# nloyfer/wgbs_tools

Measured on AMD Instinct MI355X. Metric: CpG-sites/sec segmented, higher is better.
Workload: dtype u8 counts -> u32 prefix sums -> f32/f64 log-likelihood (bit-exact with the reference)

## Files before the change

### include/wgbsseg.h

```cpp
#ifndef WGBSSEG_H
#define WGBSSEG_H

#include <stddef.h>
#include <stdint.h>

#ifdef __cplusplus
extern "C" {
#endif

#define WGBSSEG_VERSION 290
#define WGBSSEG_MAX_CPG 65535

#define WGBSSEG_OK              0
#define WGBSSEG_E_ARG          -1
#define WGBSSEG_E_METH_GT_COV  -2
#define WGBSSEG_E_NOMEM        -3
#define WGBSSEG_E_HIP          -4
#define WGBSSEG_E_LOCI_ORDER   -5
#define WGBSSEG_E_CAPACITY     -6
#define WGBSSEG_E_STATE        -7
#define WGBSSEG_E_IO           -8

typedef struct wgbsseg_ctx wgbsseg_ctx;

typedef struct wgbsseg_params {
    float    pseudo_count;
    uint32_t max_cpg;
    uint32_t max_bp;
} wgbsseg_params;

typedef struct wgbsseg_timings {
    double scan_ms;
    double window_ms;
    double cost_ms;
    double dp_ms;
    double trace_ms;
    double total_ms;
    int64_t sites;
    int64_t pairs;
    int64_t evals;
    int64_t scan_bytes;
    int32_t max_window;
    int32_t n_stages;
    int32_t scan_launches;
    int32_t div_short;
    double  scan_main_ms;
    int64_t scan_main_bytes;
} wgbsseg_timings;

int wgbsseg_version(void);

int wgbsseg_device_count(void);

int wgbsseg_create(int device, wgbsseg_ctx** out, char* err, size_t errlen);
void wgbsseg_destroy(wgbsseg_ctx* ctx);

int wgbsseg_set_betas_host(wgbsseg_ctx* ctx, const uint8_t* const* samples, int64_t n_samples, int64_t n_sites,
                           char* err, size_t errlen);
int wgbsseg_set_lbetas_host(wgbsseg_ctx* ctx, const uint16_t* const* samples, int64_t n_samples, int64_t n_sites,
                            char* err, size_t errlen);
int wgbsseg_set_betas_device(wgbsseg_ctx* ctx, const void* base, int64_t n_samples, int64_t pitch_bytes,
                             int64_t n_sites, char* err, size_t errlen);

int wgbsseg_set_loci_host(wgbsseg_ctx* ctx, const uint32_t* loci, int64_t n_sites, char* err, size_t errlen);
int wgbsseg_set_loci_device(wgbsseg_ctx* ctx, const void* loci, int64_t n_sites, char* err, size_t errlen);

int wgbsseg_segment_chunks(wgbsseg_ctx* ctx, const int64_t* chunk_start0, const int32_t* chunk_len,
                           int64_t n_chunks, const wgbsseg_params* params,
                           int32_t* borders_out, int64_t borders_cap, int64_t* borders_off,
                           char* err, size_t errlen);

int wgbsseg_segment_regions(wgbsseg_ctx* ctx, const int64_t* region_start, const int64_t* region_end, int64_t n_regions,
                            int64_t chunk_size, const wgbsseg_params* params,
                            int32_t* borders_out, int64_t borders_cap, int64_t* borders_off, int64_t* stats,
                            char* err, size_t errlen);

typedef int (*wgbsseg_batch_fn)(void* user, const int64_t* starts, const int64_t* ends, int64_t n,
                                const int32_t** out_ptr, int64_t* out_cnt);
int wgbsseg_stitch_regions(const int64_t* region_start, const int64_t* region_end, int64_t n_regions, int64_t chunk_size,
                           wgbsseg_batch_fn fn, void* user, int32_t speculate, int32_t* borders_out, int64_t borders_cap,
                           int64_t* borders_off, int64_t* stats, char* err, size_t errlen);

int wgbsseg_first_batch_items(const int64_t* region_start, const int64_t* region_end, int64_t n_regions, int64_t chunk_size,
                              int32_t speculate, int64_t* starts, int64_t* ends, int64_t cap, int64_t* n_items, int64_t* n_chunks,
                              char* err, size_t errlen);

int wgbsseg_set_site_base(wgbsseg_ctx* ctx, int64_t site_base);

typedef struct wgbsseg_group wgbsseg_group;
int wgbsseg_plan_shares(const uint32_t* loci, int64_t n_sites, const int64_t* region_start, const int64_t* region_end,
                        int64_t n_regions, int64_t chunk_size, const wgbsseg_params* params, int32_t n_shares, int64_t halo,
                        int64_t* own_lo, int64_t* own_hi, int64_t* win_lo, int64_t* win_hi, int64_t* share_chunks,
                        int64_t* share_work, char* err, size_t errlen);
// ... 68 lines not shown
                     const wgbsseg_bed_opts* opts, int fd, int64_t* lines_written, int64_t* bytes_written,
                     char* err, size_t errlen);
void wgbsseg_beta2bed_pass_ms(const wgbsseg_ctx* ctx, double* length_ms, double* emit_ms);
void wgbsseg_beta2bed_limits(int64_t* default_slab, int64_t* max_slab, int32_t* max_stage_bytes, int32_t* max_name);

int wgbsseg_site_counts(wgbsseg_ctx* ctx, const int64_t* site0, int64_t n_rows, const int32_t* samples, int32_t n_cols,
                        uint16_t* out, char* err, size_t errlen);
typedef struct {
    int32_t min_cov;
    int32_t reserved;
    int64_t slab_rows;
} wgbsseg_site_table_opts;
int wgbsseg_site_table(wgbsseg_ctx* ctx, const int64_t* site0, int64_t n_rows, const int32_t* samples, int32_t n_cols,
                       const char* labels, const int64_t* label_off, const wgbsseg_site_table_opts* opts, int fd,
                       int64_t* lines_written, int64_t* bytes_written, char* err, size_t errlen);
void wgbsseg_site_table_pass_ms(const wgbsseg_ctx* ctx, double* gather_ms, double* length_ms, double* emit_ms);
void wgbsseg_site_table_limits(int64_t* default_slab_rows, int64_t* max_slab_rows, int32_t* max_label, int32_t* max_cols);

int wgbsseg_convert_regions(wgbsseg_ctx* ctx, const int64_t* chrom_lo, const int64_t* chrom_hi, const int64_t* chrom_bp,
                            const int64_t* start, const int64_t* end, const uint8_t* slow, int64_t n,
                            int64_t* start_cpg, int64_t* end_cpg, char* err, size_t errlen);

int wgbsseg_add_loci(const uint32_t* loci, int64_t n_sites, const int64_t* chrom_cum, const char* const* chrom_names,
                     int32_t n_chroms, const int64_t* start_cpg, const int64_t* end_cpg, int64_t n_blocks,
                     const char* path, int32_t append, int32_t threads, char* err, size_t errlen);

int wgbsseg_add_loci_borders(const uint32_t* loci, int64_t n_sites, const int64_t* chrom_cum, const char* const* chrom_names,
                             int32_t n_chroms, const int32_t* borders, const int64_t* borders_off, int64_t n_regions,
                             int64_t min_cpg, const char* path, int32_t append, int32_t threads,
                             int64_t* n_written, int64_t* n_dropped, char* err, size_t errlen);

int wgbsseg_blocks_parse(const char* text, int64_t len, int64_t max_rows, int64_t cap, int64_t* line_off, int32_t* len3,
                         int64_t* start_cpg, int64_t* end_cpg, uint8_t* na, int64_t* n_rows,
                         int64_t* bp_start, int64_t* bp_end, int32_t* bp_ok, int32_t* first_fields);
int wgbsseg_blocks_write_table(const char* path, int32_t append, const char* text, const int64_t* line_off, const int32_t* len3,
                               const int64_t* start_cpg, const int64_t* end_cpg, const uint8_t* na, int64_t n_rows,
                               const double* values, int64_t n_cols, int64_t stride, int32_t digits, int32_t threads, char* err, size_t errlen);
int wgbsseg_blocks_write_bedgraph(const char* path, const char* text, const int64_t* line_off, const int32_t* len3, int64_t n_rows,
                                  const void* rows, int32_t wide, int32_t threads, char* err, size_t errlen);
int64_t wgbsseg_format_fixed(const double* v, int64_t n, int32_t digits, char* out, int64_t out_cap);

int wgbsseg_bed_parse(const char* text, int64_t len, int64_t cap, const char* const* chrom_names, int32_t n_chroms, int64_t* line_off,
                      int32_t* len3, int32_t* row_len, int32_t* chrom, int64_t* start, int64_t* end, int64_t* n_rows, int32_t* width, int32_t* header);
int64_t wgbsseg_debug_canonical_float(const char* tokens, int64_t len, uint8_t* out, int64_t out_cap);
int wgbsseg_bed_write_annotated(const char* path, const char* text, const int64_t* line_off, const int32_t* len3, const int32_t* row_len,
                                const int64_t* start_cpg, const int64_t* end_cpg, int64_t n_rows, int32_t threads, char* err, size_t errlen);

typedef struct wgbsseg_patbeta wgbsseg_patbeta;
int wgbsseg_patbeta_create(int device, int64_t start_cpg, int64_t end_cpg, wgbsseg_patbeta** out, char* err, size_t errlen);
int wgbsseg_patbeta_feed(wgbsseg_patbeta* pb, const char* text, int64_t n_bytes, char* err, size_t errlen);
int wgbsseg_patbeta_finish(wgbsseg_patbeta* pb, int32_t lbeta, void* out, char* err, size_t errlen);
void wgbsseg_patbeta_destroy(wgbsseg_patbeta* pb);
double wgbsseg_patbeta_kernel_ms(wgbsseg_patbeta* pb);

typedef struct wgbsseg_homog wgbsseg_homog;
int wgbsseg_homog_create(int device, const int64_t* start_cpg, const int64_t* end_cpg, int64_t n_blocks, const float* range, int32_t n_bins,
                         int32_t min_cpgs, int32_t inclusive, wgbsseg_homog** out, char* err, size_t errlen);
int wgbsseg_homog_feed(wgbsseg_homog* h, const char* text, int64_t n_bytes, char* err, size_t errlen);
int wgbsseg_homog_finish(wgbsseg_homog* h, int32_t* counts, char* err, size_t errlen);
void wgbsseg_homog_destroy(wgbsseg_homog* h);
double wgbsseg_homog_kernel_ms(wgbsseg_homog* h);
int wgbsseg_debug_homog_bins(const float* range, int32_t n_bins, int32_t max_total, int8_t* out);

typedef struct wgbsseg_bimodal wgbsseg_bimodal;
int wgbsseg_bimodal_create(int device, const int64_t* start_cpg, const int64_t* end_cpg, int64_t n_blocks, int32_t strict, int32_t min_len,
                           int32_t max_lds_cols, wgbsseg_bimodal** out, char* err, size_t errlen);
int wgbsseg_bimodal_feed(wgbsseg_bimodal* b, const char* text, int64_t n_bytes, char* err, size_t errlen);
int wgbsseg_bimodal_finish(wgbsseg_bimodal* b, double* ll, int64_t* counts, char* err, size_t errlen);
void wgbsseg_bimodal_destroy(wgbsseg_bimodal* b);
double wgbsseg_bimodal_kernel_ms(wgbsseg_bimodal* b);
int wgbsseg_debug_bimodal_terms(const uint32_t* a, const uint32_t* b, int64_t count, uint64_t* out);

int wgbsseg_patbeta_feed_bgzf(wgbsseg_patbeta* pb, const void* bytes, int64_t n_bytes, int64_t* consumed, char* err, size_t errlen);
int wgbsseg_homog_feed_bgzf(wgbsseg_homog* h, const void* bytes, int64_t n_bytes, int64_t* consumed, char* err, size_t errlen);
int wgbsseg_bimodal_feed_bgzf(wgbsseg_bimodal* b, const void* bytes, int64_t n_bytes, int64_t* consumed, char* err, size_t errlen);
double wgbsseg_patbeta_inflate_ms(wgbsseg_patbeta* pb);
double wgbsseg_homog_inflate_ms(wgbsseg_homog* h);
double wgbsseg_bimodal_inflate_ms(wgbsseg_bimodal* b);
int wgbsseg_bgzf_inflate(int device, const void* bytes, int64_t n_bytes, void* out, int64_t out_cap, int64_t* out_len, int64_t* consumed,
                         char* err, size_t errlen);

int wgbsseg_get_timings(const wgbsseg_ctx* ctx, wgbsseg_timings* out);

int64_t wgbsseg_debug_fetch(wgbsseg_ctx* ctx, const char* what, void* out, int64_t cap_bytes);
int wgbsseg_debug_sample_terms(wgbsseg_ctx* ctx, const float* nmeth, const float* ntotal, int64_t count,
                               float pseudo_count, float* out);
int wgbsseg_debug_log2(wgbsseg_ctx* ctx, uint32_t first_bits, int64_t count, uint32_t* out_f, uint64_t* out_d,
                       uint64_t* out_fast);
int wgbsseg_debug_div(wgbsseg_ctx* ctx, const float* a, const float* b, int64_t count, uint32_t* out_fast, uint32_t* out_ieee);
int wgbsseg_debug_check_div(wgbsseg_ctx* ctx, float pseudo_count, int32_t max_total, int64_t* mismatches);
int wgbsseg_debug_div_short(wgbsseg_ctx* ctx, const float* a, const float* b, int64_t count, uint32_t* out);

#ifdef __cplusplus
}
#endif
#endif
```

### wgbs_tools_amd/_lib.py

```python
import ctypes as C
import os
import os.path as op

import numpy as np

HERE = op.dirname(op.abspath(__file__))
LIB_PATH = op.join(HERE, 'csrc', 'libwgbsseg.so')
if os.environ.get('WGBSSEG_LIB') and os.environ.get('WGBSSEG_ALLOW_LIB_OVERRIDE') == '1':
    LIB_PATH = os.environ['WGBSSEG_LIB']
    import sys as _sys
    print('[wgbsseg] WGBSSEG_LIB: loading %s instead of the in-tree library' % LIB_PATH, file=_sys.stderr)
SYNTH_LIB_PATH = op.join(HERE, 'csrc', 'libwgbssynth.so')

OK, E_ARG, E_METH_GT_COV, E_NOMEM, E_HIP, E_LOCI_ORDER, E_CAPACITY, E_STATE, E_IO = 0, -1, -2, -3, -4, -5, -6, -7, -8

ABI_VERSION = 290
EXPORTS = ['wgbsseg_version', 'wgbsseg_device_count', 'wgbsseg_create', 'wgbsseg_destroy',
           'wgbsseg_set_betas_host', 'wgbsseg_set_betas_device', 'wgbsseg_set_loci_host', 'wgbsseg_set_loci_device',
           'wgbsseg_segment_chunks', 'wgbsseg_segment_regions', 'wgbsseg_segment_chunks_host', 'wgbsseg_prefix_sums', 'wgbsseg_scan_only',
           'wgbsseg_get_timings', 'wgbsseg_debug_fetch', 'wgbsseg_debug_sample_terms', 'wgbsseg_debug_log2',
           'wgbsseg_debug_div', 'wgbsseg_debug_check_div', 'wgbsseg_debug_div_short', 'wgbsseg_add_loci', 'wgbsseg_add_loci_borders', 'wgbsseg_block_sums', 'wgbsseg_last_block_sums_ms',
           'wgbsseg_set_site_base', 'wgbsseg_stitch_regions', 'wgbsseg_group_create', 'wgbsseg_group_destroy', 'wgbsseg_group_size',
           'wgbsseg_group_plan', 'wgbsseg_group_load_host', 'wgbsseg_group_share_set_device', 'wgbsseg_group_segment_regions', 'wgbsseg_group_segment_region_range',
           'wgbsseg_group_get_timings', 'wgbsseg_plan_shares', 'wgbsseg_set_lbetas_host',
           'wgbsseg_convert_regions', 'wgbsseg_patbeta_create', 'wgbsseg_patbeta_feed', 'wgbsseg_patbeta_finish',
           'wgbsseg_patbeta_destroy', 'wgbsseg_patbeta_kernel_ms', 'wgbsseg_group_load_host_async', 'wgbsseg_group_load_wait',
           'wgbsseg_marker_stats', 'wgbsseg_blocks_parse', 'wgbsseg_blocks_write_table', 'wgbsseg_blocks_write_bedgraph',
           'wgbsseg_format_fixed', 'wgbsseg_bed_parse', 'wgbsseg_bed_write_annotated', 'wgbsseg_debug_canonical_float',
           'wgbsseg_first_batch_items', 'wgbsseg_plan_shares_weighted',
           'wgbsseg_homog_create', 'wgbsseg_homog_feed', 'wgbsseg_homog_finish', 'wgbsseg_homog_destroy', 'wgbsseg_homog_kernel_ms',
           'wgbsseg_debug_homog_bins',
           'wgbsseg_bimodal_create', 'wgbsseg_bimodal_feed', 'wgbsseg_bimodal_finish', 'wgbsseg_bimodal_destroy', 'wgbsseg_bimodal_kernel_ms',
           'wgbsseg_debug_bimodal_terms', 'wgbsseg_sample_stats',
           'wgbsseg_pair_ranges', 'wgbsseg_pair_hist', 'wgbsseg_pair_hist_limits',
           'wgbsseg_beta2bed', 'wgbsseg_beta2bed_pass_ms', 'wgbsseg_beta2bed_limits',
           'wgbsseg_site_counts', 'wgbsseg_site_table', 'wgbsseg_site_table_pass_ms', 'wgbsseg_site_table_limits',
           'wgbsseg_patbeta_feed_bgzf', 'wgbsseg_homog_feed_bgzf', 'wgbsseg_bimodal_feed_bgzf',
           'wgbsseg_patbeta_inflate_ms', 'wgbsseg_homog_inflate_ms', 'wgbsseg_bimodal_inflate_ms', 'wgbsseg_bgzf_inflate']


class NativeLibraryError(RuntimeError):
    pass


class SegmentorError(RuntimeError):

    def __init__(self, code, msg):
        super().__init__('[wgbsseg %d] %s' % (code, msg))
        self.code = code
        self.msg = msg


class Params(C.Structure):
    _fields_ = [('pseudo_count', C.c_float), ('max_cpg', C.c_uint32), ('max_bp', C.c_uint32)]


SAMPLE_STAT_DTYPE = np.dtype([('n_sites', np.uint64), ('meth_sum', np.uint64), ('cov_sum', np.uint64), ('covered', np.uint64),
                              ('covered_at', np.uint64), ('orphans', np.uint64), ('ratio_lo', np.uint64), ('ratio_hi', np.uint64),
                              ('max_cov', np.uint32), ('reserved', np.uint32)])

PAIR_RANGE_DTYPE = np.dtype([('n', np.uint64), ('a_min', np.float64), ('a_max', np.float64), ('b_min', np.float64), ('b_max', np.float64)])


class BedOpts(C.Structure):
    _fields_ = [('min_cov', C.c_int32), ('mean', C.c_int32), ('keep_na', C.c_int32), ('stage_bytes', C.c_int32), ('slab_sites', C.c_int64)]


class SiteTableOpts(C.Structure):
    _fields_ = [('min_cov', C.c_int32), ('reserved', C.c_int32), ('slab_rows', C.c_int64)]


class Timings(C.Structure):
    _fields_ = [('scan_ms', C.c_double), ('window_ms', C.c_double), ('cost_ms', C.c_double), ('dp_ms', C.c_double),
                ('trace_ms', C.c_double), ('total_ms', C.c_double), ('sites', C.c_int64), ('pairs', C.c_int64),
                ('evals', C.c_int64), ('scan_bytes', C.c_int64), ('max_window', C.c_int32), ('n_stages', C.c_int32),
                ('scan_launches', C.c_int32), ('div_short', C.c_int32), ('scan_main_ms', C.c_double),
                ('scan_main_bytes', C.c_int64)]

    def as_dict(self):
        return {k: getattr(self, k) for k, _ in self._fields_}


BATCH_FN = C.CFUNCTYPE(C.c_int, C.c_void_p, C.POINTER(C.c_int64), C.POINTER(C.c_int64), C.c_int64, C.POINTER(C.c_void_p),
                       C.POINTER(C.c_int64))

_lib = None
_synth = None
ERRLEN = 512
_hip_preloaded = False


def _share_hip_runtime_with_torch():
    global _hip_preloaded
    if _hip_preloaded:
        return
    _hip_preloaded = True
    import importlib.util
    import sys
    if 'torch' in sys.modules:
        return
    try:
        spec = importlib.util.find_spec('torch')
    except (ImportError, ValueError):
        spec = None
    if spec is None or not spec.origin:
        return
    cand = op.join(op.dirname(spec.origin), 'lib', 'libamdhip64.so')
    if op.isfile(cand):
        try:
            C.CDLL(cand, mode=C.RTLD_GLOBAL)
        except OSError:
            pass


def load():
    global _lib
    if _lib is not None:
        return _lib
    if not op.isfile(LIB_PATH):
        raise NativeLibraryError('%s is missing: build it with `python -m wgbs_tools_amd.build` (needs hipcc). '
                                 'There is no CPU fallback.' % LIB_PATH)
    _share_hip_runtime_with_torch()
    L = C.CDLL(LIB_PATH)
    vp, i64, i32 = C.c_void_p, C.c_int64, C.c_int
    L.wgbsseg_version.restype = i32
    got = L.wgbsseg_version()
    if got != ABI_VERSION:
        raise NativeLibraryError('%s reports ABI version %d, this binding was written against %d (include/wgbsseg.h WGBSSEG_VERSION): '
                                 'rebuild it with `python -m wgbs_tools_amd.build -f`' % (LIB_PATH, got, ABI_VERSION))
    L.wgbsseg_device_count.restype = i32
    L.wgbsseg_create.restype = i32
    L.wgbsseg_create.argtypes = [i32, C.POINTER(vp), C.c_char_p, C.c_size_t]
    L.wgbsseg_destroy.restype = None
    L.wgbsseg_destroy.argtypes = [vp]
    L.wgbsseg_set_betas_host.restype = i32
    L.wgbsseg_set_betas_host.argtypes = [vp, C.POINTER(vp), i64, i64, C.c_char_p, C.c_size_t]
    L.wgbsseg_set_lbetas_host.restype = i32
    L.wgbsseg_set_lbetas_host.argtypes = [vp, C.POINTER(vp), i64, i64, C.c_char_p, C.c_size_t]
    L.wgbsseg_set_betas_device.restype = i32
    L.wgbsseg_set_betas_device.argtypes = [vp, vp, i64, i64, i64, C.c_char_p, C.c_size_t]
    L.wgbsseg_set_loci_host.restype = i32
    L.wgbsseg_set_loci_host.argtypes = [vp, vp, i64, C.c_char_p, C.c_size_t]
    L.wgbsseg_set_loci_device.restype = i32
    L.wgbsseg_set_loci_device.argtypes = [vp, vp, i64, C.c_char_p, C.c_size_t]
    L.wgbsseg_segment_chunks.restype = i32
    L.wgbsseg_segment_chunks.argtypes = [vp, vp, vp, i64, C.POINTER(Params), vp, i64, vp, C.c_char_p, C.c_size_t]
    L.wgbsseg_segment_regions.restype = i32
    L.wgbsseg_segment_regions.argtypes = [vp, vp, vp, i64, i64, C.POINTER(Params), vp, i64, vp, vp, C.c_char_p, C.c_size_t]
    L.wgbsseg_segment_chunks_host.restype = i32
    L.wgbsseg_segment_chunks_host.argtypes = [vp, i64, i64, i64, vp, vp, vp, i64, C.POINTER(Params), i32, vp, i64, vp,
                                              C.c_char_p, C.c_size_t]
    L.wgbsseg_prefix_sums.restype = i32
    L.wgbsseg_prefix_sums.argtypes = [vp, i64, i64, vp, C.c_char_p, C.c_size_t]
    L.wgbsseg_scan_only.restype = i32
    L.wgbsseg_scan_only.argtypes = [vp, vp, vp, i64, i32, i32, C.POINTER(C.c_double), C.POINTER(i64), C.POINTER(i64), C.c_char_p, C.c_size_t]
    L.wgbsseg_get_timings.restype = i32
    L.wgbsseg_get_timings.argtypes = [vp, C.POINTER(Timings)]
    L.wgbsseg_debug_fetch.restype = i64
    L.wgbsseg_debug_fetch.argtypes = [vp, C.c_char_p, vp, i64]
    L.wgbsseg_debug_sample_terms.restype = i32
    L.wgbsseg_debug_sample_terms.argtypes = [vp, vp, vp, i64, C.c_float, vp]
    L.wgbsseg_debug_log2.restype = i32
    L.wgbsseg_debug_log2.argtypes = [vp, C.c_uint32, i64, vp, vp, vp]
    L.wgbsseg_debug_div_short.restype = i32
    L.wgbsseg_debug_div_short.argtypes = [vp, vp, vp, i64, vp]
    L.wgbsseg_debug_check_div.restype = i32
    L.wgbsseg_debug_check_div.argtypes = [vp, C.c_float, i32, vp]
    L.wgbsseg_debug_div.restype = i32
    L.wgbsseg_debug_div.argtypes = [vp, vp, vp, i64, vp, vp]
    L.wgbsseg_block_sums.restype = i32
    L.wgbsseg_block_sums.argtypes = [vp, vp, vp, i64, i32, C.c_uint32, vp, C.c_char_p, C.c_size_t]
    L.wgbsseg_last_block_sums_ms.restype = C.c_double
    L.wgbsseg_last_block_sums_ms.argtypes = [vp]
    L.wgbsseg_sample_stats.restype = i32
    L.wgbsseg_sample_stats.argtypes = [vp, vp, vp, i64, i32, vp, C.c_char_p, C.c_size_t]
    L.wgbsseg_pair_ranges.restype = i32
    L.wgbsseg_pair_ranges.argtypes = [vp, vp, vp, i64, i32, vp, C.c_char_p, C.c_size_t]
    L.wgbsseg_pair_hist.restype = i32
    L.wgbsseg_pair_hist.argtypes = [vp, vp, vp, i64, i32, i32, vp, vp, C.c_char_p, C.c_size_t]
    L.wgbsseg_pair_hist_limits.restype = None
    L.wgbsseg_pair_hist_limits.argtypes = [vp, vp]
    L.wgbsseg_beta2bed.restype = i32
    L.wgbsseg_beta2bed.argtypes = [vp, i32, i64, i64, vp, vp, C.POINTER(C.c_char_p), i32, C.POINTER(BedOpts), C.c_int, vp, vp, C.c_char_p, C.c_size_t]
    L.wgbsseg_beta2bed_pass_ms.restype = None
    L.wgbsseg_beta2bed_pass_ms.argtypes = [vp, vp, vp]
    L.wgbsseg_beta2bed_limits.restype = None
    L.wgbsseg_beta2bed_limits.argtypes = [vp, vp, vp, vp]
    L.wgbsseg_site_counts.restype = i32
    L.wgbsseg_site_counts.argtypes = [vp, vp, i64, vp, i32, vp, C.c_char_p, C.c_size_t]
    L.wgbsseg_site_table.restype = i32
    L.wgbsseg_site_table.argtypes = [vp, vp, i64, vp, i32, vp, vp, C.POINTER(SiteTableOpts), C.c_int, vp, vp, C.c_char_p, C.c_size_t]
    L.wgbsseg_site_table_pass_ms.restype = None
    L.wgbsseg_site_table_pass_ms.argtypes = [vp, vp, vp, vp]
    L.wgbsseg_site_table_limits.restype = None
    L.wgbsseg_site_table_limits.argtypes = [vp, vp, vp, vp]
    L.wgbsseg_set_site_base.restype = i32
    L.wgbsseg_set_site_base.argtypes = [vp, i64]
    L.wgbsseg_stitch_regions.restype = i32
    L.wgbsseg_stitch_regions.argtypes = [vp, vp, i64, i64, BATCH_FN, vp, i32, vp, i64, vp, vp, C.c_char_p, C.c_size_t]
    L.wgbsseg_first_batch_items.restype = i32
    L.wgbsseg_first_batch_items.argtypes = [vp, vp, i64, i64, i32, vp, vp, i64, C.POINTER(i64), C.POINTER(i64), C.c_char_p, C.c_size_t]
    L.wgbsseg_plan_shares.restype = i32
    L.wgbsseg_plan_shares.argtypes = [vp, i64, vp, vp, i64, i64, C.POINTER(Params), i32, i64, vp, vp, vp, vp, vp, vp, C.c_char_p, C.c_size_t]
    L.wgbsseg_plan_shares_weighted.restype = i32
    L.wgbsseg_plan_shares_weighted.argtypes = [vp, i64, vp, vp, i64, i64, C.POINTER(Params), i32, vp, i64, vp, vp, vp, vp, vp, vp, C.c_char_p, C.c_size_t]
    L.wgbsseg_group_create.restype = i32
    L.wgbsseg_group_create.argtypes = [vp, i32, C.POINTER(vp), C.c_char_p, C.c_size_t]
    L.wgbsseg_group_destroy.restype = None
    L.wgbsseg_group_destroy.argtypes = [vp]
    L.wgbsseg_group_size.restype = i32
    L.wgbsseg_group_size.argtypes = [vp]
    L.wgbsseg_group_plan.restype = i32
    L.wgbsseg_group_plan.argtypes = [vp, vp, i64, vp, vp, i64, i64, C.POINTER(Params), i64, vp, vp, vp, vp, C.c_char_p, C.c_size_t]
    L.wgbsseg_group_load_host.restype = i32
    L.wgbsseg_group_load_host.argtypes = [vp, C.POINTER(vp), i64, i64, C.c_char_p, C.c_size_t]
    L.wgbsseg_group_load_host_async.restype = i32
    L.wgbsseg_group_load_host_async.argtypes = [vp, C.POINTER(vp), i64, i64, C.c_char_p, C.c_size_t]
    L.wgbsseg_group_load_wait.restype = i32
    L.wgbsseg_group_load_wait.argtypes = [vp, C.c_char_p, C.c_size_t]
    L.wgbsseg_group_share_set_device.restype = i32
    L.wgbsseg_group_share_set_device.argtypes = [vp, i32, vp, i64, i64, C.c_char_p, C.c_size_t]
    L.wgbsseg_group_segment_regions.restype = i32
    L.wgbsseg_group_segment_regions.argtypes = [vp, vp, i64, vp, vp, C.c_char_p, C.c_size_t]
    L.wgbsseg_group_segment_region_range.restype = i32
    L.wgbsseg_group_segment_region_range.argtypes = [vp, i64, i64, vp, i64, vp, vp, C.c_char_p, C.c_size_t]
    L.wgbsseg_group_get_timings.restype = i32
    L.wgbsseg_group_get_timings.argtypes = [vp, i32, C.POINTER(Timings)]
    L.wgbsseg_convert_regions.restype = i32
    L.wgbsseg_convert_regions.argtypes = [vp, vp, vp, vp, vp, vp, vp, i64, vp, vp, C.c_char_p, C.c_size_t]
    L.wgbsseg_patbeta_create.restype = i32
    L.wgbsseg_patbeta_create.argtypes = [i32, i64, i64, C.POINTER(vp), C.c_char_p, C.c_size_t]
    L.wgbsseg_patbeta_feed.restype = i32
    L.wgbsseg_patbeta_feed.argtypes = [vp, C.c_char_p, i64, C.c_char_p, C.c_size_t]
    L.wgbsseg_patbeta_finish.restype = i32
    L.wgbsseg_patbeta_finish.argtypes = [vp, i32, vp, C.c_char_p, C.c_size_t]
    L.wgbsseg_patbeta_destroy.restype = None
    L.wgbsseg_patbeta_destroy.argtypes = [vp]
    L.wgbsseg_patbeta_kernel_ms.restype = C.c_double
    L.wgbsseg_patbeta_kernel_ms.argtypes = [vp]
    L.wgbsseg_homog_create.restype = i32
# ... 240 lines not shown
        _check(self._L.wgbsseg_pair_ranges(self._h, a.ctypes.data, b.ctypes.data, a.size, int(min_cov), out.ctypes.data, self._err, ERRLEN), self._err)
        return out

    def pair_hist(self, pairs, min_cov, bins, edges):
        a, b = self._pair_columns(pairs)
        bins = int(bins)
        e = np.ascontiguousarray(edges, dtype=np.float64)
        if a.size and bins >= 1 and e.size != a.size * 2 * (bins + 1):
            raise ValueError('pair_hist: edges must hold [n_pairs = %d][2][bins + 1 = %d] doubles, got %d' % (a.size, bins + 1, e.size))
        counts = np.zeros((a.size, max(bins, 0), max(bins, 0)), dtype=np.uint64)
        _check(self._L.wgbsseg_pair_hist(self._h, a.ctypes.data, b.ctypes.data, a.size, int(min_cov), bins, e.ctypes.data, counts.ctypes.data,
                                         self._err, ERRLEN), self._err)
        return counts

    def beta2bed(self, fd, sample, chrom_names, chrom_cum, start0=0, end0=None, mult=None, min_cov=1, mean=False, keep_na=False,
                 slab_sites=0, stage_bytes=0):
        end0 = self.n_sites if end0 is None else int(end0)
        cum = np.ascontiguousarray(chrom_cum, dtype=np.int64)
        names = (C.c_char_p * len(chrom_names))(*[str(n).encode() for n in chrom_names])
        m = None
        if mult is not None:
            m = np.ascontiguousarray(mult, dtype=np.uint16)
            if m.size != max(end0 - int(start0), 0):
                raise ValueError('beta2bed: mult must hold one count per site of [start0, end0): %d for %d sites' % (m.size, end0 - int(start0)))
        opts = BedOpts(int(min_cov), int(bool(mean)), int(bool(keep_na)), int(stage_bytes), int(slab_sites))
        lines, nbytes = C.c_int64(0), C.c_int64(0)
        rc = self._L.wgbsseg_beta2bed(self._h, int(sample), int(start0), end0, None if m is None else m.ctypes.data, cum.ctypes.data, names,
                                      len(chrom_names), C.byref(opts), int(fd), C.addressof(lines), C.addressof(nbytes), self._err, ERRLEN)
        if rc == E_IO:
            import re
            found = re.search(r'errno (\d+)', self._err.value.decode(errors='replace'))
            code = int(found.group(1)) if found else 5
            raise OSError(code, os.strerror(code))
        _check(rc, self._err)
        return int(lines.value), int(nbytes.value)

    def beta2bed_pass_ms(self):
        a, b = C.c_double(0), C.c_double(0)
        self._L.wgbsseg_beta2bed_pass_ms(self._h, C.addressof(a), C.addressof(b))
        return float(a.value), float(b.value)

    def site_counts(self, site0, samples):
        s = np.ascontiguousarray(site0, dtype=np.int64).ravel()
        cols = np.ascontiguousarray(samples, dtype=np.int32).ravel()
        out = np.zeros((s.size, cols.size, 2), dtype=np.uint16)
        _check(self._L.wgbsseg_site_counts(self._h, s.ctypes.data, s.size, cols.ctypes.data, cols.size, out.ctypes.data, self._err, ERRLEN), self._err)
        return out

    def site_table(self, fd, site0, samples, labels, min_cov=3, slab_rows=0):
        s = np.ascontiguousarray(site0, dtype=np.int64).ravel()
        cols = np.ascontiguousarray(samples, dtype=np.int32).ravel()
        labels = [x if isinstance(x, bytes) else str(x).encode() for x in labels]
        if len(labels) != s.size:
            raise ValueError('site_table: %d labels for %d sites' % (len(labels), s.size))
        off = np.zeros(s.size + 1, dtype=np.int64)
        if labels:
            np.cumsum(np.fromiter(map(len, labels), dtype=np.int64, count=len(labels)), out=off[1:])
        blob = b''.join(labels)
        opts = SiteTableOpts(int(min_cov), 0, int(slab_rows))
        lines, nbytes = C.c_int64(0), C.c_int64(0)
        rc = self._L.wgbsseg_site_table(self._h, s.ctypes.data, s.size, cols.ctypes.data, cols.size, blob, off.ctypes.data, C.byref(opts), int(fd),
                                        C.addressof(lines), C.addressof(nbytes), self._err, ERRLEN)
        if rc == E_IO:
            import re
            found = re.search(r'errno (\d+)', self._err.value.decode(errors='replace'))
            code = int(found.group(1)) if found else 5
            raise OSError(code, os.strerror(code))
        _check(rc, self._err)
        return int(lines.value), int(nbytes.value)

    def site_table_pass_ms(self):
        a, b, c = C.c_double(0), C.c_double(0), C.c_double(0)
        self._L.wgbsseg_site_table_pass_ms(self._h, C.addressof(a), C.addressof(b), C.addressof(c))
        return float(a.value), float(b.value), float(c.value)

    def last_block_sums_ms(self):
        return float(self._L.wgbsseg_last_block_sums_ms(self._h))

    def timings(self):
        t = Timings()
        self._L.wgbsseg_get_timings(self._h, C.byref(t))
        return t.as_dict()

    def debug_fetch(self, what, dtype, count):
        out = np.empty(count, dtype=dtype)
        got = self._L.wgbsseg_debug_fetch(self._h, what.encode(), out.ctypes.data, out.nbytes)
        if got < 0:
            raise SegmentorError(int(got), 'debug_fetch(%s) failed' % what)
        return out[:got // out.itemsize]

    def debug_sample_terms(self, nmeth, ntotal, pcount):
        nmeth = np.ascontiguousarray(nmeth, dtype=np.float32)
        ntotal = np.ascontiguousarray(ntotal, dtype=np.float32)
        out = np.empty_like(nmeth)
        rc = self._L.wgbsseg_debug_sample_terms(self._h, nmeth.ctypes.data, ntotal.ctypes.data, nmeth.size,
                                                C.c_float(pcount), out.ctypes.data)
        if rc != OK:
            raise SegmentorError(rc, 'debug_sample_terms failed')
        return out

    def debug_check_div(self, pseudo_count, max_total=255 * 60):
        n = C.c_int64(0)
        rc = self._L.wgbsseg_debug_check_div(self._h, C.c_float(pseudo_count), int(max_total), C.byref(n))
        if rc != 0:
            raise SegmentorError(rc, 'debug_check_div failed')
        return int(n.value)

    def debug_div_short(self, a, b):
        a = np.ascontiguousarray(a, dtype=np.float32)
        b = np.ascontiguousarray(b, dtype=np.float32)
        out = np.empty(a.size, dtype=np.uint32)
        rc = self._L.wgbsseg_debug_div_short(self._h, a.ctypes.data, b.ctypes.data, a.size, out.ctypes.data)
        if rc != 0:
            raise SegmentorError(rc, 'debug_div_short failed')
        return out

    def debug_div(self, a, b):
        a = np.ascontiguousarray(a, dtype=np.float32)
        b = np.ascontiguousarray(b, dtype=np.float32)
        f = np.empty(a.size, dtype=np.uint32)
        g = np.empty(a.size, dtype=np.uint32)
        rc = self._L.wgbsseg_debug_div(self._h, a.ctypes.data, b.ctypes.data, a.size, f.ctypes.data, g.ctypes.data)
        if rc != OK:
            raise SegmentorError(rc, 'debug_div failed')
        return f, g

    def debug_log2(self, first_bits, count, want_f=True, want_d=True, want_fast=False):
        f = np.empty(count, dtype=np.uint32) if want_f else None
        d = np.empty(count, dtype=np.uint64) if want_d else None
        g = np.empty(count, dtype=np.uint64) if want_fast else None
        rc = self._L.wgbsseg_debug_log2(self._h, int(first_bits), int(count), f.ctypes.data if want_f else None,
                                        d.ctypes.data if want_d else None, g.ctypes.data if want_fast else None)
        if rc != OK:
            raise SegmentorError(rc, 'debug_log2 failed')
        return (f, d, g) if want_fast else (f, d)


class _PatFeed:
    _abi = None

    def __init__(self):
        self._L = load()
        self._h = C.c_void_p()
        self._err = C.create_string_buffer(ERRLEN)

    def _call(self, name, *args):
        _check(getattr(self._L, 'wgbsseg_%s_%s' % (self._abi, name))(*args, self._err, ERRLEN), self._err)

    def feed(self, text):
        self._call('feed', self._h, text, len(text))

    def feed_bgzf(self, data):
        used = C.c_int64(0)
        self._call('feed_bgzf', self._h, data, len(data), C.byref(used))
        return int(used.value)

    def inflate_ms(self):
        return float(getattr(self._L, 'wgbsseg_%s_inflate_ms' % self._abi)(self._h))

    def kernel_ms(self):
        return float(getattr(self._L, 'wgbsseg_%s_kernel_ms' % self._abi)(self._h))

    def close(self):
        if self._h:
            getattr(self._L, 'wgbsseg_%s_destroy' % self._abi)(self._h)
            self._h = C.c_void_p()
# ... 550 lines not shown
```

### wgbs_tools_amd/csrc/seg_kernels.h

```cpp
#pragma once
#include <hip/hip_runtime.h>
#include <stddef.h>
#include <stdint.h>
#include "exact_log2.h"
#include "wave_prims.h"

#ifndef WG_CARRY_SHIFT
#define WG_CARRY_SHIFT  7
#endif
#define WG_SCAN_STAGED  512
#define WG_CARRY_G      (1 << WG_CARRY_SHIFT)
static_assert(WG_CARRY_SHIFT >= 4 && WG_CARRY_SHIFT <= 10, "k_scan: a lane vector is 16 sites, an iteration 1024");
#define WG_BLOCK        256
#define WG_WIN_TILE     1024
#define WG_PAIR_CAP     4096
#define WG_TRACE_WIN    32768
#define WG_NARROW_WMAX  60
#define WG_MEDIUM_WMAX  252
#define WG_MEDIUM_TS    16

__device__ const wg_log_tables g_wg_tables = WG_LOG_TABLES_INIT;

__device__ __forceinline__ void wg_fast_tables_to_lds(wg_fast_tables* ft, int tid, int nthreads)
{
// ... 422 lines not shown
        if (k >= n) continue;
        uint32_t e = base[q] + (incl[q] - tot[q]);
#pragma unroll
        for (int x = 0; x < WG_BLOCK / 64; x++) if (x < wv) e += ws[q][x];
        const int64_t at = (int64_t)(((uint64_t)(uint32_t)info[q].y << 32) | (uint32_t)info[q].x) + k;
        uint32_t* C = cum32 + at;
        const uint4 o = make_uint4(e, e + w[q][0], e + w[q][0] + w[q][1], e + w[q][0] + w[q][1] + w[q][2]);
        if (k + 4 <= n) *reinterpret_cast<uint4*>(C) = o;
        else { C[0] = o.x; if (k + 1 < n) C[1] = o.y; if (k + 2 < n) C[2] = o.z; }
    }
}

struct PlanArgs { const int32_t* sb; int32_t TI, WA, TK, n_stages, WM; };

struct TileDesc { int32_t chunk, ka, nk, et_lo; };

__device__ __forceinline__ void wg_group_tiles(const JobView& J, const ChunkDesc& cd, const PlanArgs& P, int ka, int s1,
                                               uint32_t& nA, uint32_t& nB, uint32_t& nM)
{
    const int kb = (ka + P.TI < s1) ? ka + P.TI : s1;
    uint32_t m = 0, tb = 0, tm = 0;
    for (int k0 = ka; k0 < kb; k0 += 16) {
        const uint32_t um = J.umax16[cd.unit_off + (k0 >> 4)];
        const int nk = (kb - k0 < 16) ? kb - k0 : 16;
        m = um > m ? um : m;
        if (um <= (uint32_t)P.WM) tm += 1u;
        else tb += ((uint32_t)(nk - 1) + um + (uint32_t)P.TK - 1u) / (uint32_t)P.TK;
    }
    const bool narrow = m <= (uint32_t)P.WA;
    nA = narrow ? 1u : 0u;
    nB = narrow ? 0u : tb;
    nM = narrow ? 0u : tm;
}

__global__ __launch_bounds__(WG_BLOCK) void k_tile_count(JobView J, PlanArgs P, uint32_t* __restrict__ cntA, uint32_t* __restrict__ cntB,
                                                         uint32_t* __restrict__ cntM)
{
    __shared__ uint32_t wa[WG_BLOCK / 64], wb[WG_BLOCK / 64], wm[WG_BLOCK / 64];
    const int tid = threadIdx.x, lane = tid & 63, wv = tid >> 6;
    const int c = blockIdx.x, stg = blockIdx.y;
    const ChunkDesc cd = J.chunks[c];
    const int s0 = P.sb[stg];
    uint32_t a = 0, b = 0, m = 0;
    if (s0 < cd.len) {
        const int s1 = (P.sb[stg + 1] < cd.len) ? P.sb[stg + 1] : cd.len;
        const int nU = (s1 - s0 + P.TI - 1) / P.TI;
        for (int u = tid; u < nU; u += WG_BLOCK) {
            uint32_t na, nb, nm;
            wg_group_tiles(J, cd, P, s0 + u * P.TI, s1, na, nb, nm);
            a += na; b += nb; m += nm;
        }
    }
    for (int o = 32; o > 0; o >>= 1) { a += (uint32_t)__shfl_down((int)a, o); b += (uint32_t)__shfl_down((int)b, o); m += (uint32_t)__shfl_down((int)m, o); }
    if (lane == 0) { wa[wv] = a; wb[wv] = b; wm[wv] = m; }
    __syncthreads();
    if (tid == 0) {
        uint32_t ta = 0, tb = 0, tm = 0;
        for (int q = 0; q < WG_BLOCK / 64; q++) { ta += wa[q]; tb += wb[q]; tm += wm[q]; }
        cntA[(int64_t)stg * J.n_chunks + c] = ta;
        cntB[(int64_t)stg * J.n_chunks + c] = tb;
        cntM[(int64_t)stg * J.n_chunks + c] = tm;
    }
}

#define WG_PLAN_BLOCK 256
__global__ __launch_bounds__(WG_PLAN_BLOCK) void k_stage_plan(JobView J, PlanArgs P, const uint32_t* __restrict__ cntA,
                                                         const uint32_t* __restrict__ cntB, const uint32_t* __restrict__ cntM, int64_t* cbase, uint32_t* cum0,
                                                         int64_t* tbaseA, int64_t* tbaseB, int64_t* tbaseM, int64_t* stage_pairs, int64_t* stage_tiles)
{
    __shared__ uint64_t wa[WG_PLAN_BLOCK / 64], wb[WG_PLAN_BLOCK / 64], wc[WG_PLAN_BLOCK / 64], wd[WG_PLAN_BLOCK / 64];
    const int tid = threadIdx.x, lane = tid & 63, wv = tid >> 6;
    const int stg = blockIdx.x;
    const int nC = J.n_chunks;
    uint64_t runA = 0, runB = 0, runC = 0, runD = 0;
    for (int base = 0; base < nC; base += WG_PLAN_BLOCK) {
        const int c = base + tid;
        uint64_t sz = 0, nt = 0, nu = 0, nm = 0;
        uint32_t c0 = 0;
        if (c < nC) {
            const ChunkDesc cd = J.chunks[c];
            const int64_t s0 = P.sb[stg];
            if (s0 < cd.len) {
                const int64_t s1 = (P.sb[stg + 1] < cd.len) ? P.sb[stg + 1] : cd.len;
                c0 = J.cum32[cd.site_off + s0];
                const uint64_t cend = (s1 < cd.len) ? (uint64_t)J.cum32[cd.site_off + s1] : (uint64_t)J.chunk_pairs[c];
                sz = cend - c0;
                nt = cntA ? (uint64_t)cntA[(int64_t)stg * nC + c] : (uint64_t)((s1 - s0 + P.TI - 1) / P.TI);
                nu = cntA ? (uint64_t)cntB[(int64_t)stg * nC + c] : 0;
                nm = cntA ? (uint64_t)cntM[(int64_t)stg * nC + c] : 0;
            }
        }
        const uint64_t ia = wg_wave_incl_scan_u64(sz, lane), ib = wg_wave_incl_scan_u64(nt, lane), ic = wg_wave_incl_scan_u64(nu, lane),
                       id = wg_wave_incl_scan_u64(nm, lane);
        if (lane == 63) { wa[wv] = ia; wb[wv] = ib; wc[wv] = ic; wd[wv] = id; }
        __syncthreads();
        uint64_t oa = 0, ob = 0, oc = 0, od = 0, ta = 0, tb2 = 0, tc = 0, td = 0;
#pragma unroll
        for (int q = 0; q < WG_PLAN_BLOCK / 64; q++) {
            if (q < wv) { oa += wa[q]; ob += wb[q]; oc += wc[q]; od += wd[q]; }
            ta += wa[q]; tb2 += wb[q]; tc += wc[q]; td += wd[q];
        }
        __syncthreads();
        if (c < nC) {
            cbase[(int64_t)stg * nC + c] = (int64_t)(runA + oa + ia - sz);
            cum0[(int64_t)stg * nC + c] = c0;
            tbaseA[(int64_t)stg * (nC + 1) + c] = (int64_t)(runB + ob + ib - nt);
            tbaseB[(int64_t)stg * (nC + 1) + c] = (int64_t)(runC + oc + ic - nu);
            tbaseM[(int64_t)stg * (nC + 1) + c] = (int64_t)(runD + od + id - nm);
        }
        runA += ta; runB += tb2; runC += tc; runD += td;
    }
    if (tid == 0) {
        tbaseA[(int64_t)stg * (nC + 1) + nC] = (int64_t)runB;
        tbaseB[(int64_t)stg * (nC + 1) + nC] = (int64_t)runC;
        tbaseM[(int64_t)stg * (nC + 1) + nC] = (int64_t)runD;
        stage_pairs[stg] = (int64_t)runA;
        stage_tiles[3 * stg] = (int64_t)runB;
        stage_tiles[3 * stg + 1] = (int64_t)runC;
        stage_tiles[3 * stg + 2] = (int64_t)runD;
    }
}

__global__ __launch_bounds__(WG_BLOCK) void k_tile_emit(JobView J, PlanArgs P, int stg, const int64_t* __restrict__ tbaseA,
                                                        const int64_t* __restrict__ tbaseB, const int64_t* __restrict__ tbaseM,
                                                        TileDesc* __restrict__ tilesA, TileDesc* __restrict__ tilesB, TileDesc* __restrict__ tilesM)
{
    __shared__ uint32_t wa[WG_BLOCK / 64], wb[WG_BLOCK / 64], wm[WG_BLOCK / 64];
    const int tid = threadIdx.x, lane = tid & 63, wv = tid >> 6;
    const int c = blockIdx.x;
    const int nC = J.n_chunks;
    const ChunkDesc cd = J.chunks[c];
    const int s0 = P.sb[stg];
    if (s0 >= cd.len) return;
    const int s1 = (P.sb[stg + 1] < cd.len) ? P.sb[stg + 1] : cd.len;
    const int nU = (s1 - s0 + P.TI - 1) / P.TI;
    int64_t runA = tbaseA[(int64_t)stg * (nC + 1) + c], runB = tbaseB[(int64_t)stg * (nC + 1) + c], runM = tbaseM[(int64_t)stg * (nC + 1) + c];
    for (int base = 0; base < nU; base += WG_BLOCK) {
        const int u = base + tid;
        const int ka = s0 + u * P.TI;
        uint32_t na = 0, nb = 0, nm = 0;
        if (u < nU) wg_group_tiles(J, cd, P, ka, s1, na, nb, nm);
        const uint32_t ia = wg_wave_incl_scan_dpp_u32(na), ib = wg_wave_incl_scan_dpp_u32(nb), im = wg_wave_incl_scan_dpp_u32(nm);
        if (lane == 63) { wa[wv] = ia; wb[wv] = ib; wm[wv] = im; }
        __syncthreads();
        uint32_t oa = 0, ob = 0, om = 0, ta = 0, tb = 0, tm = 0;
#pragma unroll
        for (int q = 0; q < WG_BLOCK / 64; q++) { if (q < wv) { oa += wa[q]; ob += wb[q]; om += wm[q]; } ta += wa[q]; tb += wb[q]; tm += wm[q]; }
        __syncthreads();
        if (u < nU) {
            const int kb = (ka + P.TI < s1) ? ka + P.TI : s1;
            if (na) {
                TileDesc d = {c, ka, kb - ka, 0};
                tilesA[runA + oa + ia - na] = d;
            } else {
                int64_t o = runB + ob + ib - nb, om2 = runM + om + im - nm;
                for (int k0 = ka; k0 < kb; k0 += 16) {
                    const uint32_t um = J.umax16[cd.unit_off + (k0 >> 4)];
                    const int nk = (kb - k0 < 16) ? kb - k0 : 16;
                    if (um <= (uint32_t)P.WM) { TileDesc d = {c, k0, nk, 0}; tilesM[om2++] = d; continue; }
                    const int kt = (int)(((uint32_t)(nk - 1) + um + (uint32_t)P.TK - 1u) / (uint32_t)P.TK);
                    for (int e = 0; e < kt; e++) { TileDesc d = {c, k0, nk, k0 + e * P.TK}; tilesB[o++] = d; }
                }
            }
        }
        runA += ta; runB += tb; runM += tm;
    }
}

struct CostArgs {
    float pc, pc2;
    int32_t NS;
    int32_t rows;
    const wg_d2* tab;
    int32_t xcd_group;
    int32_t cmap;
    uint32_t* finished;
};

__global__ __launch_bounds__(64) void k_stage_gate(const uint32_t* __restrict__ finished, uint32_t need, long long max_ticks)
{
    if (threadIdx.x != 0) return;
    const long long t0 = wall_clock64();
    while (__hip_atomic_load(finished, __ATOMIC_RELAXED, __HIP_MEMORY_SCOPE_AGENT) < need && wall_clock64() - t0 < max_ticks) __builtin_amdgcn_s_sleep(8);
}

__device__ __forceinline__ void wg_stage_prefix_row(uint2* __restrict__ dst, const uint8_t* __restrict__ row,
                                                    const uint2* __restrict__ carry, const ChunkDesc& cd,
                                                    int64_t n_total, int A, int x0, int cnt0, int lane)
{
    const int cnt = x0 + cnt0;
    const int64_t abs0 = cd.start0 + A;
    const uint2 c0 = carry[(abs0 >> WG_CARRY_SHIFT) - (cd.start0 >> WG_CARRY_SHIFT)];
    uint32_t run_m = c0.x, run_t = c0.y;
    const int64_t al = abs0 & ~3LL;
    const int hs = (int)(abs0 - al);
    for (int p0 = 0; p0 < cnt + hs; p0 += 256) {
        const int sidx = p0 + lane * 4;
        const int64_t a = al + sidx;
        uint32_t w0 = 0, w1 = 0;
        if (sidx < cnt + hs) {
            if (a + 4 <= n_total) {
                const uint2 v = *reinterpret_cast<const uint2*>(row + 2 * a);
                w0 = v.x; w1 = v.y;
            } else {
                for (int j = 0; j < 4; j++) if (a + j < n_total) {
                    const uint32_t h = (uint32_t)row[2 * (a + j)] | ((uint32_t)row[2 * (a + j) + 1] << 8);
                    if (j < 2) w0 |= h << (16 * j); else w1 |= h << (16 * (j - 2));
                }
            }
        }
        uint32_t m[4], t[4];
        uint32_t tot = 0;
#pragma unroll
        for (int j = 0; j < 4; j++) {
            const uint32_t h = ((j < 2) ? w0 : w1) >> (16 * (j & 1));
            const int x = sidx + j - hs;
            const bool in = x >= 0 && (A + x) < cd.len;
            m[j] = in ? (h & 0xffu) : 0u;
            t[j] = in ? ((h >> 8) & 0xffu) : 0u;
            tot += m[j] | (t[j] << 16);
        }
        const uint32_t incl = wg_wave_incl_scan_dpp_u32(tot);
        const uint32_t excl = incl - tot;
        uint32_t em = run_m + (excl & 0xffffu), et = run_t + (excl >> 16);
#pragma unroll
        for (int j = 0; j < 4; j++) {
            const int x = sidx + j - hs;
            if (x >= x0 && x < cnt) dst[x - x0] = make_uint2(em, et);
            em += m[j]; et += t[j];
        }
        const uint32_t wt = (uint32_t)__builtin_amdgcn_readlane((int)incl, 63);
        run_m += wt & 0xffffu; run_t += wt >> 16;
    }
}

__device__ __forceinline__ int wg_group_start(const ChunkDesc& cd, int k)
{
    const int64_t a = (cd.start0 + k) & ~(int64_t)(WG_CARRY_G - 1);
    return a <= cd.start0 ? 0 : (int)(a - cd.start0);
}

template <int ROW>
__device__ __forceinline__ void wg_stage_local_rows(uint32_t* __restrict__ Et, const uint8_t* __restrict__ betas, int64_t pitch,
                                                    int s_first, int ns, const ChunkDesc& cd, int64_t n_total, int ka, int cnt,
                                                    int lane, int wv)
{
    constexpr bool WHOLE = ROW > 128;
    const int half = WHOLE ? 0 : lane >> 5, l5 = WHOLE ? lane : lane & 31;
    const int64_t abs0 = cd.start0 + ka;
    const int64_t al = abs0 & ~3LL;
    const int hs = (int)(abs0 - al);
    const int sidx = l5 * 4;
    const int64_t a = al + sidx;
    const int nsite = cnt - 1;
    for (int r0 = WHOLE ? wv : wv * 2; r0 < ns; r0 += (WHOLE ? 1 : 2) * (WG_BLOCK / 64)) {
        const int rr = r0 + half;
        const bool act = rr < ns;
        uint32_t w0 = 0, w1 = 0;
        if (act && sidx < nsite + hs) {
            const uint8_t* row = betas + (int64_t)(s_first + rr) * pitch;
// ... 39 lines not shown
    const int hs = (int)(abs0 - al);
    const int nsite = cnt - 1;
    for (int rr = wv; rr < ns; rr += WG_BLOCK / 64) {
        const uint8_t* row = betas + (int64_t)(s_first + rr) * pitch;
        uint32_t* dst = Et + (size_t)rr * ROW;
        uint32_t run = 0;
        for (int p0 = 0; p0 < nsite + hs; p0 += 256) {
            const int sidx = p0 + lane * 4;
            const int64_t a = al + sidx;
            uint32_t w0 = 0, w1 = 0;
            if (sidx < nsite + hs) {
                if (a + 4 <= n_total) {
                    const uint2 v = *reinterpret_cast<const uint2*>(row + 2 * a);
                    w0 = v.x; w1 = v.y;
                } else {
                    for (int j = 0; j < 4; j++) if (a + j < n_total) {
                        const uint32_t h = (uint32_t)row[2 * (a + j)] | ((uint32_t)row[2 * (a + j) + 1] << 8);
                        if (j < 2) w0 |= h << (16 * j); else w1 |= h << (16 * (j - 2));
                    }
                }
            }
            uint32_t mt[4];
            uint32_t tot = 0;
#pragma unroll
            for (int j = 0; j < 4; j++) {
                const uint32_t h = ((j < 2) ? w0 : w1) >> (16 * (j & 1));
                const int x = sidx + j - hs;
                const bool in = x >= 0 && x < nsite;
                mt[j] = in ? ((h & 0xffu) | ((h & 0xff00u) << 8)) : 0u;
                tot += mt[j];
            }
            const uint32_t incl = wg_wave_incl_scan_dpp_u32(tot);
            uint32_t e = run + (incl - tot);
#pragma unroll
            for (int j = 0; j < 4; j++) {
                const int x = sidx + j - hs;
                if (x >= 0 && x < cnt) dst[x] = e;
                e += mt[j];
            }
            run += (uint32_t)__builtin_amdgcn_readlane((int)incl, 63);
        }
        if (lane == 0 && ((nsite + hs) & 255) == 0 && nsite < cnt) dst[nsite] = run;
    }
}

#define WG_WIDE_TK      128
#define WG_WIDE_TS      16

template <int TI, int FAST, int SPLIT, bool ONEG>
__global__ __launch_bounds__(WG_BLOCK) void k_cost(JobView J, StageView SV, CostArgs A, const TileDesc* __restrict__ tiles,
                                                   int64_t n_tiles, double* __restrict__ cost, int64_t n_tiles_padded)
{
    constexpr bool WIDE = SPLIT == 1;
    constexpr int WM = SPLIT == 2 ? WG_MEDIUM_WMAX : WG_NARROW_WMAX;
    static_assert(SPLIT != 2 || TI == WG_MEDIUM_TS, "a medium tile is one 16-site unit");
    constexpr int KS = WIDE ? WG_WIDE_TK + 1 : TI + WM + 1;
    constexpr int IS = WIDE ? WG_WIDE_TS + 1 : 0;
    constexpr bool KY = (FAST >= 2);
    constexpr bool DIVS = (FAST == 3);
    extern __shared__ __attribute__((aligned(16))) char smem[];
    static_assert(sizeof(wg_fast_tables) % 16 == 0 && sizeof(wg_d2) == 16, "the arrays behind the tables are 16-byte aligned");
    const size_t TB = KY ? (size_t)A.rows * (16 + 64) * sizeof(wg_d2) : sizeof(wg_fast_tables);
    wg_fast_tables* tb = reinterpret_cast<wg_fast_tables*>(smem);
    wg_d2* iyt = reinterpret_cast<wg_d2*>(smem);
    wg_d2* kyt = iyt + (size_t)A.rows * 16;
    const wg_d2* iy0 = iyt + (A.rows - 1) * 16;
    const wg_d2* ky0 = kyt + (A.rows - 1) * 64;
    uint2* Et = reinterpret_cast<uint2*>(smem + TB);
    uint2* St = Et + (size_t)A.NS * KS;
    uint32_t* Lt = reinterpret_cast<uint32_t*>(smem + TB);
    char* after = WIDE ? reinterpret_cast<char*>(St + (((size_t)A.NS * (KS + IS) + 1) & ~(size_t)1) - (size_t)A.NS * KS)
                       : reinterpret_cast<char*>(Lt + (((size_t)A.NS * KS + 3) & ~(size_t)3));
    struct Rec { int32_t offs, ea; int64_t sb; };
    Rec* rec = reinterpret_cast<Rec*>(after);
    int32_t* misc = reinterpret_cast<int32_t*>(rec + (TI + 1));
    uint8_t* cmap = reinterpret_cast<uint8_t*>(misc + 8);
    constexpr bool CMAP = !WIDE;

    const int tid = threadIdx.x, lane = tid & 63, wv = tid >> 6;
    const int nC = J.n_chunks;
    const int64_t G = A.xcd_group, jx = (int64_t)(blockIdx.x >> 3);
    const int64_t t = (jx / G) * (8 * G) + (int64_t)(blockIdx.x & 7) * G + (jx % G);
    if (t >= n_tiles) return;
    const TileDesc td = tiles[t];
    const int c = td.chunk;
    const ChunkDesc cd = J.chunks[c];
    const int ka = td.ka, nk = td.nk, kb = ka + nk;
    const int et_lo = WIDE ? td.et_lo : 0;
    const int et_hi = WIDE ? et_lo + WG_WIDE_TK : (1 << 30);
    const uint32_t cum0 = SV.cum0[(int64_t)SV.stage * nC + c];

    if (KY) wg_lookup_tables_to_lds(iyt, kyt, A.rows, A.tab, tid, WG_BLOCK);
    else wg_fast_tables_to_lds(tb, tid, WG_BLOCK);
    constexpr int PW = (TI + 63) / 64;
    if (wv < PW) {
        const int kl = wv * 64 + lane;
        const int k = ka + kl;
        const bool valid = kl < nk;
        int cnt = 0, is = 0, ie = -1;
        if (valid) {
            const int f = J.W16[cd.site_off + k];
            is = k > et_lo ? k : et_lo;
            ie = (k + f < et_hi ? k + f : et_hi) - 1;
            cnt = ie - is + 1;
            if (cnt < 0) cnt = 0;
        }
        const uint32_t incl = wg_wave_incl_scan_dpp_u32((uint32_t)cnt);
        if (kl < TI) {
            const int32_t o = (int32_t)(incl - (uint32_t)cnt);
            Rec r;
            r.offs = o;
            r.ea = is - o + 1 - (WIDE ? 0 : ka);
            r.sb = (valid ? (int64_t)(J.cum32[cd.site_off + k] - cum0) - k : 0) + (is - o);
            rec[kl] = r;
        }
        const uint32_t imin = wg_wave_min_u32(cnt > 0 ? (uint32_t)is : 0x7fffffffu);
        const uint32_t imax = wg_wave_max_u32(cnt > 0 ? (uint32_t)ie : 0u);
        if (lane == 0) { misc[2 * wv] = (int32_t)imin; misc[2 * wv + 1] = (int32_t)imax; }
        if (lane == 63) misc[4 + wv] = (int32_t)incl;
    }
    __syncthreads();
    const int imin = PW > 1 ? (misc[0] < misc[2] ? misc[0] : misc[2]) : misc[0];
    const int imax = PW > 1 ? (misc[1] > misc[3] ? misc[1] : misc[3]) : misc[1];
    const int Q = PW > 1 ? misc[4] + misc[5] : misc[4];
    if (Q == 0) { if (A.finished != nullptr && tid == 0) __hip_atomic_fetch_add(A.finished, 1u, __ATOMIC_RELAXED, __HIP_MEMORY_SCOPE_AGENT); return; }
    const int eA = WIDE ? imin + 1 : ka;
    if (PW > 1 || WIDE) {
        if (wv < PW && wv * 64 + lane < TI) {
            const int t0 = wv == 1 ? misc[4] : 0;
            Rec& r = rec[wv * 64 + lane];
            if (PW > 1 && wv == 1) { r.offs += t0; r.sb -= t0; }
            if (WIDE || (PW > 1 && wv == 1)) r.ea -= t0 + (WIDE ? eA : 0);
        }
    }
    if (PW > 1 || WIDE) __syncthreads();
    if (tid == 0) rec[nk].offs = Q;
    if (CMAP && tid < nk) {
        const int o0 = rec[tid].offs, o1 = tid + 1 < nk ? rec[tid + 1].offs : Q;
        const int sh = A.cmap;
        for (int g = (o0 + (1 << sh) - 1) >> sh; (g << sh) < o1; g++) cmap[g] = (uint8_t)tid;
    }
    const int eG = wg_group_start(cd, eA < cd.len ? eA : cd.len - 1);
    const int Ecnt = imax + 2 - eA;
    const int sG = wg_group_start(cd, ka);
    const int Scnt = kb - ka;

    const float pc = A.pc, pc2 = A.pc2;
    double* cb = cost + SV.cbase[(int64_t)SV.stage * nC + c];
    static_assert(TI <= 64 || ONEG, "128-start tiles hold every sample at once");
    constexpr bool ONEGROUP = ONEG;
    double accR[ONEGROUP ? 1 : WG_PAIR_CAP / WG_BLOCK];
    for (int g0 = 0; g0 < J.n_samples; g0 += A.NS) {
        const int ns = (J.n_samples - g0 < A.NS) ? J.n_samples - g0 : A.NS;
        const bool firstg = ONEGROUP || g0 == 0, lastg = ONEGROUP || g0 + ns >= J.n_samples;
        __syncthreads();
        if (WIDE) {
            for (int rr = wv; rr < ns; rr += WG_BLOCK / 64) {
                const int s = g0 + rr;
                const uint8_t* row = J.betas + (int64_t)s * J.pitch;
                const uint2* carry = J.carry + cd.carry_off + (int64_t)s * cd.nG;
                wg_stage_prefix_row(Et + (size_t)rr * KS, row, carry, cd, J.n_total, eG, eA - eG, Ecnt, lane);
                wg_stage_prefix_row(St + (size_t)rr * IS, row, carry, cd, J.n_total, sG, ka - sG, Scnt, lane);
            }
        } else if (SPLIT == 2) {
            wg_stage_local_rows_long<KS>(Lt, J.betas, J.pitch, g0, ns, cd, J.n_total, ka, Ecnt, lane, wv);
        } else {
// ... 1059 lines not shown
```

### wgbs_tools_amd/csrc/wgbsseg.hip

```cpp
#include <hip/hip_runtime.h>
#include <algorithm>
#include <atomic>
#include <cerrno>
#include <chrono>
#include <cstdarg>
#include <cstdio>
#include <cstdlib>
#include <cstring>
#include <deque>
#include <functional>
#include <initializer_list>
#include <memory>
#include <string>
#include <thread>
#include <type_traits>
#include <vector>
#include <pthread.h>
#include <sched.h>
#include <sys/mman.h>
#include <unistd.h>
#if defined(__x86_64__) && !defined(__HIP_DEVICE_COMPILE__)
#include <emmintrin.h>
#endif

// ... 45 lines not shown
}

#define WG_MAX_CPUS 8192
struct NearCpus { std::vector<unsigned long> bits; bool valid = false; };

enum BatchEvent { EV_BEGIN, EV_WINDOWS, EV_SCAN_END, EV_PLAN, EV_TRACE0, EV_TRACE1, EV_HOME, EV_STATS, EV_VALIDATE0, EV_VALIDATE1, EV_SCAN0, EV_SCAN1, EV_UPLOADED, EV_COUNT };

struct BedScratch {
    DevBuf tab, mult, wg, out[2];
    PinnedBuf home[2], tot;
    struct PassEvents { Event len0, len1, emit0, emit1; } ev[2];
    double len_ms = 0.0, emit_ms = 0.0;
};

struct SiteScratch {
    DevBuf site0, samples, labels, label_off, cells;
    struct GatherEvents { Event g0, g1; } ev[2];
    double gather_ms = 0.0, len_ms = 0.0, emit_ms = 0.0;
};

struct wgbsseg_ctx {
    int device = 0;
    NearCpus near_cpus;
    Stream sA, sB, sC;
    Stream sA2;
    DevBuf betas_own, loci_own;
    const uint8_t* betas = nullptr;
    int64_t pitch = 0, n_total = 0;
    int32_t elem = 1;
    int64_t site_base = 0;
    int32_t n_samples = 0;
    const uint32_t* loci = nullptr;
    int64_t n_loci = 0;
    DevBuf chunks, wtile, carry, W16, cum32, back16, chunk_pairs, status, tile_tot, tile_base, tile_chunk;
    DevBuf plan_cbase, plan_cum0, plan_tbase, plan_pairs, plan_tiles, plan_cnt, umax16;
    std::vector<PinnedBuf> pinned;
    std::vector<PinnedBuf> up_stage;
    DevBuf tiles[3], cost[3], stage_ctr, dpstate, tmp_borders, nb, boff, out_borders[2], edges, lookup;
    DevBuf dbg_a, dbg_b, dbg_c;
    int out_par = 0;
    Event evS;
    Event evD;
    bool out_pending = false;
    bool batch_open = false;
    std::vector<wg_d2> h_lookup;
    float lookup_pc = -1.0f;
    int lookup_rows[3] = {-1, -1, -1};
    Event ev[EV_COUNT];
    PinnedBuf h_status;
    PinnedBuf h_job, h_pieces, h_sb;
    PinnedBuf h_out;
    std::vector<Event> ev_cost0, ev_cost1, ev_dp0, ev_dp1, ev_fork, ev_join;
    wgbsseg_timings tim = {};
    int64_t last_sites = 0, last_pairs = 0;
    int32_t last_stages = 0;
    bool last_valid = false;
    long long cost_budget_bytes = 0;
    int force_stages = 0;
    bool counted_live = false;
    double stage_gate_wide_evals = 100000.0, stage_min_evals_per_step = 21000.0;
    bool stage_gate_shared = false;
    int stage_gate = 768, last_stage_pct = -1, force_dp_mode = 0, force_ns = 0, force_ti = 0;
    double last_block_sums_ms = 0.0;
    int64_t table_blocks = 0;
    bool accumulate = false;
    std::vector<std::pair<int64_t, int64_t>> validated;
    DevBuf scan_pieces, divcheck, plan_sb;
    DevBuf bs_plan, bs_desc, bs_out;
    DevBuf mk_out, cv_in, cv_out;
    DevBuf st_ranges, st_parts;
    DevBuf ph_pairs, ph_edges, ph_out;
    BedScratch bed;
    SiteScratch site;
    std::vector<int32_t> h_stage_bounds;
    float divs_pc = -1.0f;
    bool divs_ok = false;
    int64_t last_dp_chunks = 0, last_dp_stride = 0;
    float divs_m_pc = -1.0f;
    bool divs_m_ok = false;
    bool divs_enabled = true, bs_general = false;
    int64_t scan_piece_sites = 4096;
    int medium_wmax = WG_MEDIUM_WMAX;
    bool dp_wlean = true, early = true, speculate = true, batch_marks = false;
    ~wgbsseg_ctx() { (void)hipSetDevice(device); (void)hipDeviceSynchronize(); }
};

namespace {

bool device_local_cpus(int device, NearCpus* out)
{
    out->valid = false;
    if (!env_flag("WGBSSEG_UPLOAD_PIN", true)) return false;
    char bus[64] = {0};
    if (hipDeviceGetPCIBusId(bus, (int)sizeof bus, device) != hipSuccess) { (void)hipGetLastError(); return false; }
    for (char* q = bus; *q; q++) if (*q >= 'A' && *q <= 'F') *q = (char)(*q - 'A' + 'a');
    char path[160];
    snprintf(path, sizeof path, "/sys/bus/pci/devices/%s/local_cpulist", bus);
    FILE* f = fopen(path, "r");
    if (!f) return false;
    char line[8192] = {0};
    const bool got = fgets(line, (int)sizeof line, f) != nullptr;
    fclose(f);
    if (!got) return false;
    const size_t bytes = CPU_ALLOC_SIZE(WG_MAX_CPUS);
    std::vector<unsigned long> allowed(bytes / sizeof(unsigned long), 0ul);
    out->bits.assign(bytes / sizeof(unsigned long), 0ul);
    cpu_set_t* A = reinterpret_cast<cpu_set_t*>(allowed.data());
    cpu_set_t* L = reinterpret_cast<cpu_set_t*>(out->bits.data());
    if (sched_getaffinity(0, bytes, A) != 0) return false;
    int n_local = 0;
    for (const char* q = line; *q;) {
        while (*q == ',' || *q == ' ' || *q == '\n') q++;
        if (*q < '0' || *q > '9') break;
        char* end = nullptr;
        long a = strtol(q, &end, 10), b = a;
        if (*end == '-') b = strtol(end + 1, &end, 10);
        for (long x = a; x <= b && x < WG_MAX_CPUS; x++) if (CPU_ISSET_S((int)x, bytes, A)) { CPU_SET_S((int)x, bytes, L); n_local++; }
        q = end;
    }
    if (n_local == 0 || n_local == CPU_COUNT_S(bytes, A)) return false;
    out->valid = true;
    return true;
}
inline void pin_to(const NearCpus& n)
{
    if (n.valid) (void)pthread_setaffinity_np(pthread_self(), n.bits.size() * sizeof(unsigned long), reinterpret_cast<const cpu_set_t*>(n.bits.data()));
}
struct FillMode { bool populate = true, nt = true; };
inline void fill_piece(void* dst, const uint8_t* src, size_t n, const FillMode& m)
{
#ifdef MADV_POPULATE_READ
    if (m.populate) {
        const uintptr_t a = reinterpret_cast<uintptr_t>(src) & ~(uintptr_t)4095, b = (reinterpret_cast<uintptr_t>(src) + n + 4095) & ~(uintptr_t)4095;
        (void)madvise(reinterpret_cast<void*>(a), b - a, MADV_POPULATE_READ);
    }
#endif
#if defined(__x86_64__) && !defined(__HIP_DEVICE_COMPILE__)
    if (m.nt && (reinterpret_cast<uintptr_t>(dst) & 15) == 0) {
        __m128i* d = reinterpret_cast<__m128i*>(dst);
        const __m128i* s = reinterpret_cast<const __m128i*>(src);
        size_t v = n >> 6;
        for (; v > 0; v--, s += 4, d += 4) {
            const __m128i x0 = _mm_loadu_si128(s), x1 = _mm_loadu_si128(s + 1), x2 = _mm_loadu_si128(s + 2), x3 = _mm_loadu_si128(s + 3);
            _mm_stream_si128(d, x0); _mm_stream_si128(d + 1, x1); _mm_stream_si128(d + 2, x2); _mm_stream_si128(d + 3, x3);
        }
        _mm_sfence();
        const size_t done = n & ~(size_t)63;
        if (n > done) memcpy(static_cast<char*>(dst) + done, src + done, n - done);
        return;
    }
#endif
    memcpy(dst, src, n);
}
struct UploadPlan {
    int64_t piece = 0, ppr = 0, n_tasks = 0;
    int T = 1, depth = 2;
    bool piece_major = false;
    FillMode fill = {false, false};
};
UploadPlan plan_upload(bool streaming, int64_t n_rows, int64_t row_bytes)
{
    UploadPlan u;
    const int64_t bytes = row_bytes * n_rows;
    const bool big = streaming && bytes >= (4LL << 30);
    const long long kb = env_int("WGBSSEG_UPLOAD_PIECE_KB", 0), threads = env_int("WGBSSEG_UPLOAD_THREADS", 0);
    u.piece = kb >= 64 ? (int64_t)kb << 10 : streaming ? (big ? 2 << 20 : 1 << 20) : 4 << 20;
// ... 103 lines not shown
    if (profiling()) fprintf(stderr, "[wgbsseg] betas to the device (streaming): %.1f ms, %.1f GB/s (%d upload threads x %d pieces of %lld KB%s%s%s)\n", (wall_s() - t0) * 1e3,
                             (double)row_bytes * n_rows / (wall_s() - t0) * 1e-9, u.T, u.depth, (long long)(u.piece >> 10), c->near_cpus.valid ? ", on the device's CPUs" : "",
                             u.fill.populate ? ", pages mapped per piece" : "", u.fill.nt ? ", non-temporal fill" : "");
    return WGBSSEG_OK;
}

}

extern "C" {

int wgbsseg_version(void) { return WGBSSEG_VERSION; }

int wgbsseg_device_count(void)
{
    int n = 0;
    if (hipGetDeviceCount(&n) != hipSuccess) return 0;
    return n;
}

}
namespace {
std::atomic<int> g_live_ctx[64];

int check_device(int device, char* err, size_t errlen)
{
    int n = 0;
    hipError_t e = hipGetDeviceCount(&n);
    if (e != hipSuccess || n <= 0) {
        set_err(err, errlen, "no HIP device available (%s); libwgbsseg has no CPU fallback", hipGetErrorString(e));
        return WGBSSEG_E_HIP;
    }
    if (device < 0 || device >= n) { set_err(err, errlen, "device %d out of range (0..%d)", device, n - 1); return WGBSSEG_E_ARG; }
    HIP_TRY(hipSetDevice(device));
    hipDeviceProp_t prop;
    HIP_TRY(hipGetDeviceProperties(&prop, device));
    if (!strstr(prop.gcnArchName, "gfx950")) {
        set_err(err, errlen, "device %d is %s; this library carries gfx950 code only", device, prop.gcnArchName);
        return WGBSSEG_E_HIP;
    }
    return WGBSSEG_OK;
}

int create_ctx(int device, bool scan_low_priority, wgbsseg_ctx** out, char* err, size_t errlen)
{
    if (!out) { set_err(err, errlen, "out is NULL"); return WGBSSEG_E_ARG; }
    *out = nullptr;
    const int rc = check_device(device, err, errlen);
    if (rc != WGBSSEG_OK) return rc;
    HIP_TRY(set_kernel_attributes());
    std::unique_ptr<wgbsseg_ctx> c(new (std::nothrow) wgbsseg_ctx());
    if (!c) { set_err(err, errlen, "out of host memory"); return WGBSSEG_E_NOMEM; }
    c->device = device;
    (void)device_local_cpus(device, &c->near_cpus);
    HIP_TRY(c->sA.create());
    {
        int lo_p = 0, hi_p = 0;
        (void)hipDeviceGetStreamPriorityRange(&lo_p, &hi_p);
        HIP_TRY(c->sB.create(hi_p));
        HIP_TRY(scan_low_priority ? c->sC.create(lo_p) : c->sC.create());
    }
    HIP_TRY(c->sA2.create());
    HIP_TRY(c->evD.create(false));
    HIP_TRY(c->evS.create(false));
    for (auto& v : c->ev) HIP_TRY(v.create());
    const long long budget_mb = env_int("WGBSSEG_COST_BUDGET_MB", 0);
    c->cost_budget_bytes = (budget_mb > 0 ? budget_mb : 6144LL) << 20;
    c->force_stages = (int)env_int("WGBSSEG_FORCE_STAGES", 0);
    c->stage_gate = (int)env_int("WGBSSEG_STAGE_GATE", c->stage_gate, 0);
    c->stage_gate_shared = env_flag("WGBSSEG_STAGE_GATE_SHARED", false);
    c->stage_gate_wide_evals = env_double("WGBSSEG_STAGE_GATE_WIDE_EVALS", c->stage_gate_wide_evals);
    c->stage_min_evals_per_step = env_double("WGBSSEG_STAGE_MIN_EVALS", c->stage_min_evals_per_step);
    if (env_int("WGBSSEG_LAST_STAGE_PCT", -1) != -1) c->last_stage_pct = (int)env_int("WGBSSEG_LAST_STAGE_PCT", -1, 5, 800);
    c->force_dp_mode = (int)env_int("WGBSSEG_DP_MODE", 0, 0, 2);
    c->force_ns = (int)env_int("WGBSSEG_NS", 0);
    c->force_ti = (int)env_int("WGBSSEG_TI", 0);
    c->bs_general = env_flag("WGBSSEG_BLOCK_SUMS_GENERAL", false);
    c->divs_enabled = env_flag("WGBSSEG_DIV_SHORT", true);
    { const long long sp = env_int("WGBSSEG_SCAN_PIECE_SITES", 0); if (sp >= 1024) c->scan_piece_sites = sp & ~1023LL; }
    const int wm = (int)env_int("WGBSSEG_MEDIUM_WMAX", WG_MEDIUM_WMAX, 0, WG_MEDIUM_WMAX);
    c->medium_wmax = wm > WG_NARROW_WMAX ? wm : 0;
    c->dp_wlean = env_flag("WGBSSEG_DP_WLEAN", true);
    c->early = !env_flag("WGBSSEG_NO_EARLY", false);
    c->speculate = !env_flag("WGBSSEG_NO_SPECULATION", false);
    c->batch_marks = env_int("WGBSSEG_PROFILE", 0) >= 2;
    g_live_ctx[device & 63].fetch_add(1, std::memory_order_relaxed);
    c->counted_live = true;
    *out = c.release();
    return WGBSSEG_OK;
}
}
extern "C" {

int wgbsseg_create(int device, wgbsseg_ctx** out, char* err, size_t errlen) { return create_ctx(device, true, out, err, errlen); }

void wgbsseg_destroy(wgbsseg_ctx* c)
{
    if (!c) return;
    if (c->counted_live) g_live_ctx[c->device & 63].fetch_sub(1, std::memory_order_relaxed);
    const double t0 = wall_s();
    delete c;
    if (profiling()) fprintf(stderr, "[wgbsseg] destroy: %.1f ms\n", (wall_s() - t0) * 1e3);
}

static hipError_t own_rows(wgbsseg_ctx* c, int64_t n_samples, int64_t n_sites, int elem)
{
    const int64_t pitch = round_up(2 * elem * n_sites, 256) + 256;
    const hipError_t e = c->betas_own.ensure((size_t)pitch * (size_t)n_samples);
    if (e != hipSuccess) return e;
    c->betas = c->betas_own.as<uint8_t>();
    c->pitch = pitch; c->n_total = n_sites; c->n_samples = (int32_t)n_samples; c->elem = elem;
    c->last_valid = false;
    return hipSuccess;
}

static int set_rows_host(wgbsseg_ctx* c, const uint8_t* const* samples, int64_t n_samples, int64_t n_sites, int elem, char* err, size_t errlen)
{
    if (!c || !samples || n_samples < 1 || n_sites < 1) { set_err(err, errlen, "bad arguments to set_betas_host"); return WGBSSEG_E_ARG; }
    for (int64_t s = 0; s < n_samples; s++)
        if (!samples[s]) { set_err(err, errlen, "samples[%lld] is NULL", (long long)s); return WGBSSEG_E_ARG; }
    HIP_TRY(hipSetDevice(c->device));
    HIP_TRY(own_rows(c, n_samples, n_sites, elem));
    return upload_rows(c, c->betas_own.as<uint8_t>(), c->pitch, samples, n_samples, 2 * elem * n_sites, "betas", err, errlen);
}

int wgbsseg_set_betas_host(wgbsseg_ctx* c, const uint8_t* const* samples, int64_t n_samples, int64_t n_sites,
                           char* err, size_t errlen)
{
    return set_rows_host(c, samples, n_samples, n_sites, 1, err, errlen);
}

int wgbsseg_set_lbetas_host(wgbsseg_ctx* c, const uint16_t* const* samples, int64_t n_samples, int64_t n_sites,
                            char* err, size_t errlen)
{
    return set_rows_host(c, reinterpret_cast<const uint8_t* const*>(samples), n_samples, n_sites, 2, err, errlen);
}

int wgbsseg_set_betas_device(wgbsseg_ctx* c, const void* base, int64_t n_samples, int64_t pitch_bytes, int64_t n_sites,
                             char* err, size_t errlen)
{
    if (!c || !base || n_samples < 1 || n_sites < 1 || pitch_bytes < 2 * n_sites) { set_err(err, errlen, "bad arguments to set_betas_device"); return WGBSSEG_E_ARG; }
    if (((uintptr_t)base & 15) || (pitch_bytes & 15)) { set_err(err, errlen, "device betas base and pitch must be multiples of 16 bytes"); return WGBSSEG_E_ARG; }
    c->betas = reinterpret_cast<const uint8_t*>(base);
    c->pitch = pitch_bytes; c->n_total = n_sites; c->n_samples = (int32_t)n_samples; c->elem = 1;
    c->last_valid = false;
    return WGBSSEG_OK;
}

int wgbsseg_set_loci_host(wgbsseg_ctx* c, const uint32_t* loci, int64_t n_sites, char* err, size_t errlen)
{
    if (!c || !loci || n_sites < 1) { set_err(err, errlen, "bad arguments to set_loci_host"); return WGBSSEG_E_ARG; }
    HIP_TRY(hipSetDevice(c->device));
    HIP_TRY(c->loci_own.ensure((size_t)n_sites * 4));
    const uint8_t* row = reinterpret_cast<const uint8_t*>(loci);
    const int rc = upload_rows(c, c->loci_own.as<uint8_t>(), 0, &row, 1, n_sites * 4, "loci", err, errlen);
    if (rc != WGBSSEG_OK) return rc;
    c->loci = c->loci_own.as<uint32_t>();
    c->n_loci = n_sites;
    c->last_valid = false;
    return WGBSSEG_OK;
}

int wgbsseg_set_loci_device(wgbsseg_ctx* c, const void* loci, int64_t n_sites, char* err, size_t errlen)
{
    if (!c || !loci || n_sites < 1) { set_err(err, errlen, "bad arguments to set_loci_device"); return WGBSSEG_E_ARG; }
    if ((uintptr_t)loci & 3) { set_err(err, errlen, "device loci must be a multiple of 4 bytes"); return WGBSSEG_E_ARG; }
    c->loci = reinterpret_cast<const uint32_t*>(loci);
    c->n_loci = n_sites;
    c->last_valid = false;
    return WGBSSEG_OK;
}

}

namespace {

struct Job {
    std::vector<ChunkDesc> h;
    std::vector<ScanPiece> pieces;
    int64_t val_sites = 0;
    std::vector<int64_t> wtile_off;
    int64_t sites = 0, carry_entries = 0, units = 0, n_hint = 0;
    int64_t sites_padded = 0;
    int32_t max_len = 0;
    JobStatus st0;
    JobView v = {};
};

int build_job(wgbsseg_ctx* c, const int64_t* start0, const int32_t* len, int64_t n_chunks, Job& job, bool need_loci,
              char* err, size_t errlen)
{
    if (!c) { set_err(err, errlen, "ctx is NULL"); return WGBSSEG_E_ARG; }
    if (!c->betas) { set_err(err, errlen, "betas not set"); return WGBSSEG_E_STATE; }
    if (c->elem != 1) { set_err(err, errlen, "the resident rows are uint16 (.lbeta): segment, scan and prefix sums read uint8 .beta data only (as the reference's segmentor, segmentor.cpp:166-176)"); return WGBSSEG_E_STATE; }
    if (need_loci && (!c->loci || c->n_loci != c->n_total)) { set_err(err, errlen, "loci not set or length differs from the betas (%lld vs %lld)", (long long)c->n_loci, (long long)c->n_total); return WGBSSEG_E_STATE; }
    if (!start0 || !len || n_chunks < 1 || n_chunks > 0x7fffffff) { set_err(err, errlen, "bad chunk list"); return WGBSSEG_E_ARG; }
    job.h.resize((size_t)n_chunks);
    job.wtile_off.resize((size_t)n_chunks + 1);
    int64_t so = 0, co = 0, wt = 0, uo = 0, total = 0;
    for (int64_t i = 0; i < n_chunks; i++) {
        if (len[i] < 1 || len[i] > (1 << 30) || start0[i] < 0 || start0[i] + len[i] > c->n_total) {
            set_err(err, errlen, "chunk %lld = [%lld, +%d) is empty or outside the %lld sites of the beta files",
                    (long long)i, (long long)start0[i], (int)len[i], (long long)c->n_total);
            return WGBSSEG_E_ARG;
        }
        ChunkDesc& d = job.h[(size_t)i];
        d.start0 = start0[i]; d.len = len[i]; d.site_off = so; d.carry_off = co; d.unit_off = uo; d.nG = (int32_t)(((start0[i] + len[i] - 1) >> WG_CARRY_SHIFT) - (start0[i] >> WG_CARRY_SHIFT) + 1);
        job.wtile_off[(size_t)i] = wt;
        wt += (len[i] + WG_WIN_TILE - 1) / WG_WIN_TILE;
        so += round_up((int64_t)len[i], 8);
        total += len[i];
        uo += (len[i] + 15) / 16;
        co += (int64_t)d.nG * c->n_samples;
        job.max_len = std::max(job.max_len, len[i]);
    }
    job.wtile_off[(size_t)n_chunks] = wt;
    {
        const int64_t nh = (wt >> 8) + 2;
        job.n_hint = nh;
        job.wtile_off.resize((size_t)n_chunks + 1 + (size_t)((nh + 1) / 2));
        int32_t* hint = reinterpret_cast<int32_t*>(job.wtile_off.data() + n_chunks + 1);
        int64_t cix = 0;
        for (int64_t h = 0; h < nh; h++) {
            const int64_t tile = h << 8;
            while (cix + 1 < n_chunks && job.wtile_off[(size_t)cix + 1] <= tile) cix++;
            hint[h] = (int32_t)cix;
        }
    }
    job.sites = total; job.sites_padded = so; job.carry_entries = co; job.units = uo;
    HIP_TRY(hipSetDevice(c->device));
    HIP_TRY(c->chunks.ensure(sizeof(ChunkDesc) * (size_t)n_chunks));
    HIP_TRY(c->carry.ensure(sizeof(uint2) * (size_t)co));
    HIP_TRY(c->status.ensure(sizeof(JobStatus)));
    HIP_TRY(c->wtile.ensure(8 * job.wtile_off.size()));
    memset(&job.st0, 0, sizeof(job.st0));
    job.st0.first_bad = ~0ULL;
    const size_t b_chunks = sizeof(ChunkDesc) * (size_t)n_chunks, b_wtile = 8 * job.wtile_off.size();
    const size_t o_wtile = (size_t)round_up((int64_t)b_chunks, 64), o_status = o_wtile + (size_t)round_up((int64_t)b_wtile, 64), o_end = o_status + 64;
    if (c->h_job.ensure(o_end)) {
        char* h = reinterpret_cast<char*>(c->h_job.p);
        memcpy(h, job.h.data(), b_chunks);
        memcpy(h + o_wtile, job.wtile_off.data(), b_wtile);
        memcpy(h + o_status, &job.st0, sizeof(job.st0));
        HIP_TRY(hipMemcpyAsync(c->chunks.p, h, b_chunks, hipMemcpyHostToDevice, c->sA));
        HIP_TRY(hipMemcpyAsync(c->wtile.p, h + o_wtile, b_wtile, hipMemcpyHostToDevice, c->sA));
        HIP_TRY(hipMemcpyAsync(c->status.p, h + o_status, sizeof(job.st0), hipMemcpyHostToDevice, c->sA));
    } else {
        HIP_TRY(hipMemcpyAsync(c->chunks.p, job.h.data(), b_chunks, hipMemcpyHostToDevice, c->sA));
        HIP_TRY(hipMemcpyAsync(c->wtile.p, job.wtile_off.data(), b_wtile, hipMemcpyHostToDevice, c->sA));
        HIP_TRY(hipMemcpyAsync(c->status.p, &job.st0, sizeof(job.st0), hipMemcpyHostToDevice, c->sA));
    }
    JobView& v = job.v;
    v.betas = c->betas; v.pitch = c->pitch; v.n_total = c->n_total; v.loci = c->loci;
    v.chunks = c->chunks.as<ChunkDesc>(); v.carry = c->carry.as<uint2>();
    v.n_samples = c->n_samples; v.n_chunks = (int32_t)n_chunks;
    return WGBSSEG_OK;
}

bool interval_covered(const std::vector<std::pair<int64_t, int64_t>>& v, int64_t lo, int64_t hi)
{
    auto it = std::upper_bound(v.begin(), v.end(), lo, [](int64_t x, const std::pair<int64_t, int64_t>& iv) { return x < iv.first; });
    return it != v.begin() && (--it)->second >= hi;
}

int plan_validation(wgbsseg_ctx* c, Job& job, bool fresh_call, char* err, size_t errlen)
{
    if (fresh_call) c->validated.clear();
    std::vector<std::pair<int64_t, int64_t>> runs;
    bool sorted = true;
    for (const ChunkDesc& d : job.h) {
        const int64_t lo = d.start0, hi = d.start0 + d.len;
        if (!runs.empty() && lo == runs.back().second) { runs.back().second = hi; continue; }
        if (interval_covered(c->validated, lo, hi) || (sorted && interval_covered(runs, lo, hi))) continue;
        if (!runs.empty() && lo < runs.back().first) sorted = false;
        runs.emplace_back(lo, hi);
    }
    const int64_t P = c->scan_piece_sites;
    job.pieces.clear(); job.val_sites = 0;
    for (const auto& r : runs) {
        job.val_sites += r.second - r.first;
        for (int64_t a = r.first; a < r.second; ) {
            const int64_t b = std::min(r.second, (a / P + 1) * P);
            job.pieces.push_back(ScanPiece{a, (int32_t)(b - a), 0});
            a = b;
        }
    }
    if (!runs.empty()) {
        std::vector<std::pair<int64_t, int64_t>>& V = c->validated;
        V.insert(V.end(), runs.begin(), runs.end());
        std::sort(V.begin(), V.end());
        size_t w = 0;
        for (size_t i = 1; i < V.size(); i++) {
            if (V[i].first <= V[w].second) V[w].second = std::max(V[w].second, V[i].second);
            else V[++w] = V[i];
        }
        V.resize(w + 1);
        HIP_TRY(c->scan_pieces.ensure(sizeof(ScanPiece) * job.pieces.size()));
        const size_t b_pieces = sizeof(ScanPiece) * job.pieces.size();
        const void* src = job.pieces.data();
        if (c->h_pieces.ensure(b_pieces)) { memcpy(c->h_pieces.p, src, b_pieces); src = c->h_pieces.p; }
        HIP_TRY(hipMemcpyAsync(c->scan_pieces.p, src, b_pieces, hipMemcpyHostToDevice, c->sA));
    }
    return WGBSSEG_OK;
}

int launch_validate(wgbsseg_ctx* c, const Job& job, hipStream_t s, char* err, size_t errlen)
{
    if (job.pieces.empty()) return WGBSSEG_OK;
    const int64_t tasks = (int64_t)job.pieces.size() * job.v.n_samples;
    const int64_t vb = (tasks + (WG_BLOCK / 64) - 1) / (WG_BLOCK / 64);
// ... 228 lines not shown
            if (score > top) { top = score; pick = ns; }
        }
        return pick;
    };
    p.NS[1] = pick_ns(1, WG_WIDE_TS, 4, true);
    p.NS[2] = pick_ns(2, WG_MEDIUM_TS, 5, false);
    const int tile_ti[3] = {p.TI, WG_WIDE_TS, WG_MEDIUM_TS};
    for (int k = 0; k < 3; k++) p.lds[k] = (size_t)round_up((int64_t)cost_lds(p, tile_ti[k], k, p.NS[k]), 16);
    return WGBSSEG_OK;
}

void plan_stages(wgbsseg_ctx* c, const Job& job, const JobStatus& st, BatchPlan& p)
{
    const int64_t total_pairs = (int64_t)st.total_pairs;
    const long long bytes = total_pairs * 8;
    int n_stages = (int)std::max<long long>(1, (bytes + c->cost_budget_bytes - 1) / c->cost_budget_bytes);
    int n_long = 0;
    for (const ChunkDesc& d : job.h) n_long += d.len >= 8192;
    const bool worth = (double)total_pairs * c->n_samples >= (double)job.max_len * c->stage_min_evals_per_step;
    if (job.max_len >= 8192) n_stages = std::max(n_stages, n_long <= 160 && worth ? 8 : 1);
    if (c->force_stages > 0) n_stages = c->force_stages;
    n_stages = std::min<int>(n_stages, std::max(1, (job.max_len + 63) / 64));
    p.all_narrow = p.Wmax <= WG_NARROW_WMAX;
    const double evals_per_step = (double)total_pairs * c->n_samples / std::max<double>(1.0, (double)job.max_len);
    p.gated = c->stage_gate > 0 && n_stages > 1 && (p.all_narrow || evals_per_step >= c->stage_gate_wide_evals || c->stage_gate_shared) &&
              (c->stage_gate_shared || g_live_ctx[c->device & 63].load(std::memory_order_relaxed) == 1);
    p.last_pct = !p.gated ? 100 : (c->last_stage_pct > 0 ? c->last_stage_pct : (evals_per_step <= 52500.0 ? 300 : 100));
    const double parts = n_stages > 1 ? (double)(n_stages - 1) + p.last_pct / 100.0 : 1.0;
    const int S = (int)round_up((int64_t)std::ceil((double)job.max_len / parts), 64);
    n_stages = std::min<int>(n_stages, (job.max_len + S - 1) / S);
    std::vector<int32_t>& sb = c->h_stage_bounds;
    sb.resize((size_t)n_stages + 1);
    for (int q = 0; q < n_stages; q++) sb[(size_t)q] = (int32_t)std::min<int64_t>((int64_t)q * S, job.max_len);
    sb[(size_t)n_stages] = (int32_t)job.max_len;
    p.sb = sb.data();
    p.n_stages = n_stages;
    p.stage_pairs.assign((size_t)n_stages, 0);
    p.stage_tiles.assign((size_t)n_stages * 3, 0);
    if (p.all_narrow) {
        for (int stg = 0; stg < n_stages; stg++) {
            int64_t nt = 0, sites_in = 0;
            for (const ChunkDesc& d : job.h) {
                const int64_t s0 = sb[(size_t)stg], s1 = std::min<int64_t>(sb[(size_t)stg + 1], d.len);
                if (s1 > s0) { nt += (s1 - s0 + p.TI - 1) / p.TI; sites_in += s1 - s0; }
            }
            p.stage_tiles[3 * (size_t)stg] = nt;
            p.stage_pairs[(size_t)stg] = n_stages == 1 ? total_pairs : std::min<int64_t>(total_pairs, sites_in * std::max(p.Wmax, 1));
        }
    }
    p.nbuf = n_stages > 1 ? (p.gated && n_stages > 2 ? 3 : 2) : 1;
    p.dp_mode = std::max(p.Wmax > 512 ? 2 : (p.Wmax > 64 ? 1 : 0), c->force_dp_mode);
    p.ringN = p.dp_mode ? ceil_pow2(p.Wmax + 128) : 0;
    p.state_stride = round_up(WG_DP_STATE_HDR + (int64_t)p.ringN + (p.ringN + 1) / 2, 2);
}

int queue_div_check(wgbsseg_ctx* c, float pc, int wmax, void* dst, char* err, size_t errlen)
{
    HIP_TRY(c->divcheck.ensure(4));
    HIP_TRY(hipMemsetAsync(c->divcheck.p, 0, 4, c->sA));
    const int max_total = 255 * wmax;
    hipLaunchKernelGGL(k_check_div, dim3((unsigned)max_total + 1), dim3(WG_BLOCK), 0, c->sA, pc, pc + pc, max_total, c->divcheck.as<unsigned int>());
    HIP_TRY(hipGetLastError());
    HIP_TRY(hipMemcpyAsync(dst, c->divcheck.p, 4, hipMemcpyDeviceToHost, c->sA));
    return WGBSSEG_OK;
}

struct Batch {
    wgbsseg_ctx* c = nullptr;
    const int64_t* chunk_start0 = nullptr; const int32_t* chunk_len = nullptr; int64_t n_chunks = 0;
    const BorderAlloc* alloc = nullptr; int64_t* borders_off = nullptr; EarlyOut* early = nullptr;
    bool allow_plain = true;
    wgbsseg_params P = {};
    Job job;
    int nC = 0; int64_t J = 0;
    JobStatus* hst = nullptr;
    JobStatus st = {};
    BatchPlan plan;
    CostArgs ca[3];
    std::vector<int64_t> tile0[3];
    DevBuf* outb = nullptr; size_t out_head = 0;
    bool marks = false;
    double hm[8] = {0, 0, 0, 0, 0, 0, 0, 0};
    void mark(int i) { if (marks) hm[i] = wall_s(); }

    int front(char* err, size_t errlen);
    int disorder_exit(char* err, size_t errlen);
    int tile_plan(char* err, size_t errlen);
    int stages(char* err, size_t errlen);
    int deliver(char* err, size_t errlen);
    int timings(char* err, size_t errlen);
};

int segment_chunks_impl(wgbsseg_ctx* c, const int64_t* chunk_start0, const int32_t* chunk_len, int64_t n_chunks,
                        const wgbsseg_params* P, const BorderAlloc& alloc, int64_t* borders_off, char* err, size_t errlen, bool allow_plain = true, EarlyOut* early = nullptr)
{
    if (!P || !borders_off) { set_err(err, errlen, "NULL params/borders pointer"); return WGBSSEG_E_ARG; }
    if (P->max_bp == 0) { set_err(err, errlen, "max_bp must be >= 1 (the reference reads uninitialised loci when it is 0: segmentor.cpp:38,114)"); return WGBSSEG_E_ARG; }
    if (P->max_cpg < 1) { set_err(err, errlen, "max_cpg must be >= 1"); return WGBSSEG_E_ARG; }
    int32_t longest = 1;
    if (chunk_len) for (int64_t i = 0; i < n_chunks; i++) longest = std::max(longest, chunk_len[i]);
    Batch b;
    b.c = c; b.chunk_start0 = chunk_start0; b.chunk_len = chunk_len; b.n_chunks = n_chunks;
    b.alloc = &alloc; b.borders_off = borders_off; b.early = early; b.allow_plain = allow_plain;
    b.P = *P;
    b.P.max_cpg = std::min<uint32_t>(P->max_cpg, (uint32_t)longest);
    if ((uint64_t)b.P.max_cpg * 255u >= (1u << 24) || b.P.max_cpg > WGBSSEG_MAX_CPG) {
        set_err(err, errlen, "max_cpg %u with chunks of up to %d sites unsupported: blocks of more than %d sites (255 * sites >= 2^24) do not keep their counts exact "
                "in the float sums of the reference itself (segmentor.cpp:122-123), and windows are stored in 16 bits", P->max_cpg, (int)longest, WGBSSEG_MAX_CPG);
        return WGBSSEG_E_ARG;
    }
    b.marks = c && c->batch_marks;
    b.mark(0);
    if (!(P->pseudo_count >= 0.0f)) { set_err(err, errlen, "pseudo_count must be >= 0"); return WGBSSEG_E_ARG; }
    if (c && c->batch_open) {
        HIP_TRY(hipSetDevice(c->device));
        HIP_TRY(hipDeviceSynchronize());
        c->out_pending = false;
    }
    if (c) c->batch_open = true;
    int rc = build_job(c, chunk_start0, chunk_len, n_chunks, b.job, true, err, errlen);
    if (rc != WGBSSEG_OK) return rc;
    rc = plan_validation(c, b.job, !c->accumulate, err, errlen);
    if (rc != WGBSSEG_OK) return rc;
    c->last_valid = false;
    b.nC = (int)n_chunks;
    b.J = b.job.sites;

    rc = b.front(err, errlen);
    if (rc != WGBSSEG_OK) return rc;
    if (b.st.loci_disorder || b.st.overflow) return b.disorder_exit(err, errlen);
    rc = plan_tiles(c, b.job, b.st, b.P.pseudo_count, b.plan, err, errlen);
    if (rc != WGBSSEG_OK) return rc;
    plan_stages(c, b.job, b.st, b.plan);
    rc = b.tile_plan(err, errlen);
    if (rc == WGBSSEG_OK) rc = b.stages(err, errlen);
    if (rc == WGBSSEG_OK) rc = b.deliver(err, errlen);
    if (rc == WGBSSEG_OK) rc = b.timings(err, errlen);
    return rc;
}

int Batch::front(char* err, size_t errlen)
{
    JobView& v = job.v;
    const int64_t Jp = job.sites_padded;
    const int64_t nT = job.wtile_off[(size_t)nC];
    if (nT > 0x7fffffff) { set_err(err, errlen, "too many sites in one call"); return WGBSSEG_E_ARG; }
    HIP_TRY(c->W16.ensure((size_t)Jp * 2 + 16));
    HIP_TRY(c->cum32.ensure((size_t)Jp * 4 + 16));
    HIP_TRY(c->back16.ensure((size_t)Jp * 2 + 16));
    HIP_TRY(c->chunk_pairs.ensure((size_t)nC * 8));
    HIP_TRY(c->umax16.ensure((size_t)job.units * 2));
    HIP_TRY(c->tile_tot.ensure((size_t)nT * 4));
    HIP_TRY(c->tile_base.ensure((size_t)nT * 4));
    HIP_TRY(c->tile_chunk.ensure((size_t)nT * 16));
    v.W16 = c->W16.as<uint16_t>(); v.cum32 = c->cum32.as<uint32_t>(); v.back16 = c->back16.as<uint16_t>();
    v.chunk_pairs = c->chunk_pairs.as<int64_t>(); v.umax16 = c->umax16.as<uint16_t>();
    if (!c->h_status.ensure(4 * sizeof(JobStatus))) { set_err(err, errlen, "out of page-locked host memory"); return WGBSSEG_E_NOMEM; }
    hst = reinterpret_cast<JobStatus*>(c->h_status.p);

    mark(1);
    HIP_TRY(hipEventRecord(c->ev[EV_BEGIN], c->sA));
    HIP_TRY(hipEventRecord(c->ev[EV_UPLOADED], c->sA));
    HIP_TRY(hipStreamWaitEvent(c->sC, c->ev[EV_UPLOADED], 0));
    HIP_TRY(hipEventRecord(c->ev[EV_VALIDATE0], c->sC));
    int rc = launch_validate(c, job, c->sC, err, errlen);
    if (rc != WGBSSEG_OK) return rc;
    HIP_TRY(hipEventRecord(c->ev[EV_VALIDATE1], c->sC));

    const bool check_div = c->divs_enabled && wg_term_mode(P.pseudo_count) == 2 && c->divs_pc != P.pseudo_count;
    if (check_div && (rc = queue_div_check(c, P.pseudo_count, WG_NARROW_WMAX, hst + 1, err, errlen)) != WGBSSEG_OK) return rc;
    int top_step = 1;
    while (2 * (int64_t)top_step <= (int64_t)P.max_cpg - 1) top_step *= 2;
    const int64_t win_want = 1 + (int64_t)WG_WIN_TILE + 2 * (int64_t)std::max(top_step, 32) + 8;
    const int win_lds = win_want <= 12288 ? (int)win_want : 0;
    const int64_t* const d_wtile = c->wtile.as<int64_t>();
    hipLaunchKernelGGL(k_window, dim3((unsigned)nT), dim3(WG_BLOCK), (size_t)win_lds * 4, c->sA, v, c->status.as<JobStatus>(),
                       d_wtile, reinterpret_cast<const int32_t*>(d_wtile + nC + 1), P.max_cpg, P.max_bp, win_lds, top_step, std::max(c->medium_wmax, WG_NARROW_WMAX),
                       c->tile_tot.as<uint32_t>(), c->tile_chunk.as<int4>());
    HIP_TRY(hipGetLastError());
    hipLaunchKernelGGL(k_window_scan, dim3((unsigned)nC), dim3(WG_BLOCK), 0, c->sA, v, c->status.as<JobStatus>(), d_wtile, c->tile_tot.as<uint32_t>(), c->tile_base.as<uint32_t>());
    HIP_TRY(hipGetLastError());
    HIP_TRY(hipEventRecord(c->ev[EV_WINDOWS], c->sA));
    HIP_TRY(hipMemcpyAsync(&hst[0], c->status.p, sizeof(JobStatus), hipMemcpyDeviceToHost, c->sA));
    HIP_TRY(hipEventRecord(c->ev[EV_STATS], c->sA));
    hipLaunchKernelGGL(k_window_cum, dim3((unsigned)((nT + WG_CUM_TILES - 1) / WG_CUM_TILES)), dim3(WG_BLOCK), 0, c->sA, (const uint16_t*)v.W16, v.cum32, (const int4*)c->tile_chunk.as<int4>(),
                       (const uint32_t*)c->tile_base.as<uint32_t>(), nT);
    HIP_TRY(hipGetLastError());
    mark(2);
    HIP_TRY(hipEventSynchronize(c->ev[EV_STATS]));
    mark(3);
    st = hst[0];
    if (check_div) {
        c->divs_ok = *reinterpret_cast<const unsigned int*>(&hst[1]) == 0u;
        c->divs_pc = P.pseudo_count;
        if (profiling()) fprintf(stderr, "[wgbsseg] short division core for pseudo count %g: %s\n", (double)P.pseudo_count, c->divs_ok ? "verified on every operand pair of a narrow tile" : "NOT exact, the full core stays");
    }
    if (st.wide_units && !st.loci_disorder && !st.overflow) {
        HIP_TRY(hipStreamWaitEvent(c->sC, c->ev[EV_WINDOWS], 0));
        HIP_TRY(hipEventRecord(c->ev[EV_SCAN0], c->sC));
        rc = launch_scan(c, job, c->sC, err, errlen);
        if (rc != WGBSSEG_OK) return rc;
        HIP_TRY(hipEventRecord(c->ev[EV_SCAN1], c->sC));
    }
    HIP_TRY(hipEventRecord(c->ev[EV_SCAN_END], c->sC));
    HIP_TRY(hipMemcpyAsync(&hst[2], c->status.p, sizeof(JobStatus), hipMemcpyDeviceToHost, c->sC));
    HIP_TRY(hipEventRecord(c->evS, c->sC));
    return WGBSSEG_OK;
}

int Batch::disorder_exit(char* err, size_t errlen)
{
    JobStatus st2;
    HIP_TRY(hipStreamSynchronize(c->sC));
    HIP_TRY(hipStreamSynchronize(c->sA));
    HIP_TRY(hipMemcpyAsync(&st2, c->status.p, sizeof(st2), hipMemcpyDeviceToHost, c->sA));
    HIP_TRY(hipStreamSynchronize(c->sA));
    if (st2.first_bad != ~0ULL) return report_bad_site(c, st2, err, errlen);
    if (!st.loci_disorder) { set_err(err, errlen, "a chunk scores more than 2^32 blocks; use a smaller chunk_size"); return WGBSSEG_E_ARG; }
    if (!allow_plain) {
        set_err(err, errlen, "internal: loci not ascending inside chunk %u (0-based sites [%lld, +%d)) of a batch that was filtered for such chunks",
                st.loci_disorder - 1, (long long)(job.h[st.loci_disorder - 1].start0 + c->site_base), (int)job.h[st.loci_disorder - 1].len);
        return WGBSSEG_E_LOCI_ORDER;
    }
    DevBuf flags;
    HIP_TRY(flags.ensure((size_t)n_chunks * 4));
    HIP_TRY(hipMemsetAsync(flags.p, 0, (size_t)n_chunks * 4, c->sA));
    hipLaunchKernelGGL(k_find_disorder, dim3((unsigned)n_chunks), dim3(WG_BLOCK), 0, c->sA, job.v, flags.as<uint32_t>());
    HIP_TRY(hipGetLastError());
    std::vector<uint32_t> hf((size_t)n_chunks);
    HIP_TRY(hipMemcpyAsync(hf.data(), flags.p, (size_t)n_chunks * 4, hipMemcpyDeviceToHost, c->sA));
    HIP_TRY(hipStreamSynchronize(c->sA));
    std::vector<int64_t> os, ooff;
    std::vector<int32_t> ol, ob;
    for (int64_t i = 0; i < n_chunks; i++) if (!hf[(size_t)i]) { os.push_back(chunk_start0[i]); ol.push_back(chunk_len[i]); }
    if (!os.empty()) {
        ooff.resize(os.size() + 1);
        const int rc = segment_chunks_impl(c, os.data(), ol.data(), (int64_t)os.size(), &P,
                                           [&](int64_t total) { ob.resize((size_t)std::max<int64_t>(1, total)); return ob.data(); }, ooff.data(), err, errlen, false);
        if (rc != WGBSSEG_OK) return rc;
    }
    std::vector<std::vector<int32_t>> plain((size_t)n_chunks);
    for (int64_t i = 0; i < n_chunks; i++)
        if (hf[(size_t)i]) {
            wgbsseg_params Pc = P;
            const int rc = plain_segment_chunk(c, chunk_start0[i], chunk_len[i], &Pc, plain[(size_t)i], err, errlen);
            if (rc != WGBSSEG_OK) return rc;
        }
    int64_t total = 0;
    size_t oi = 0;
    for (int64_t i = 0; i < n_chunks; i++) {
        borders_off[i] = total;
        if (hf[(size_t)i]) total += (int64_t)plain[(size_t)i].size();
        else { total += ooff[oi + 1] - ooff[oi]; oi++; }
    }
    borders_off[n_chunks] = total;
    int32_t* out = (*alloc)(total);
    if (!out) { set_err(err, errlen, "borders_out too small: need %lld ints", (long long)total); return WGBSSEG_E_CAPACITY; }
    oi = 0;
    for (int64_t i = 0; i < n_chunks; i++) {
        if (hf[(size_t)i]) memcpy(out + borders_off[i], plain[(size_t)i].data(), plain[(size_t)i].size() * 4);
        else { memcpy(out + borders_off[i], ob.data() + ooff[oi], (size_t)(ooff[oi + 1] - ooff[oi]) * 4); oi++; }
    }
    c->last_valid = false;
    return WGBSSEG_OK;
}

int Batch::tile_plan(char* err, size_t errlen)
{
    BatchPlan& p = plan;
    const float pc = P.pseudo_count;
    const int n_stages = p.n_stages;
    CostArgs base;
    memset(&base, 0, sizeof(base));
    base.pc = pc; base.pc2 = pc + pc;
    base.xcd_group = 64;
    base.cmap = 3;
    for (int k = 0; k < 3; k++) { ca[k] = base; ca[k].NS = p.NS[k]; ca[k].rows = p.rows[k]; }
    if (p.term_mode[0] == 2) {
        const bool same = c->lookup_pc == pc && c->lookup_rows[0] == p.rows[0] && c->lookup_rows[1] == p.rows[1] && c->lookup_rows[2] == p.rows[2] && c->lookup.p;
        if (!same) {
            static const wg_log_tables host_tabs = WG_LOG_TABLES_INIT;
            c->h_lookup.resize((size_t)(p.rows[0] + p.rows[1] + p.rows[2]) * 80);
            wg_d2* dst = c->h_lookup.data();
            for (int rows : p.rows) {
                for (int x = 0; x < rows * 16; x++) dst[x] = wg_ks_iy_entry(&host_tabs, rows, x);
                for (int x = 0; x < rows * 64; x++) dst[rows * 16 + x] = wg_ks_ky_entry(&host_tabs, rows, x);
                dst += (size_t)rows * 80;
            }
            HIP_TRY(c->lookup.ensure(c->h_lookup.size() * sizeof(wg_d2)));
            HIP_TRY(hipMemcpyAsync(c->lookup.p, c->h_lookup.data(), c->h_lookup.size() * sizeof(wg_d2), hipMemcpyHostToDevice, c->sA));
            c->lookup_pc = pc;
            for (int k = 0; k < 3; k++) c->lookup_rows[k] = p.rows[k];
        }
        const wg_d2* tab = c->lookup.as<wg_d2>();
        for (int k = 0; k < 3; k++) { ca[k].tab = tab; tab += (size_t)p.rows[k] * 80; }
    }
    const size_t sb_bytes = (size_t)(n_stages + 1) * 4;
    HIP_TRY(c->plan_sb.ensure(sb_bytes));
    const void* src = p.sb;
    if (c->h_sb.ensure(sb_bytes)) { memcpy(c->h_sb.p, src, sb_bytes); src = c->h_sb.p; }
    HIP_TRY(hipMemcpyAsync(c->plan_sb.p, src, sb_bytes, hipMemcpyHostToDevice, c->sA));
    HIP_TRY(c->plan_cbase.ensure((size_t)n_stages * nC * 8));
    HIP_TRY(c->plan_cum0.ensure((size_t)n_stages * nC * 4));
    HIP_TRY(c->plan_tbase.ensure((size_t)n_stages * (nC + 1) * 8 * 3));
    HIP_TRY(c->plan_cnt.ensure((size_t)n_stages * nC * 4 * 3));
    HIP_TRY(c->plan_pairs.ensure((size_t)n_stages * 8));
    HIP_TRY(c->plan_tiles.ensure((size_t)n_stages * 8 * 3));
    PlanArgs pa = {c->plan_sb.as<int32_t>(), p.TI, p.WA, WG_WIDE_TK, n_stages, p.WMED};
    uint32_t* cntA = c->plan_cnt.as<uint32_t>();
    uint32_t* cntB = cntA + (size_t)n_stages * nC;
    uint32_t* cntM = cntB + (size_t)n_stages * nC;
    int64_t* tbaseA = c->plan_tbase.as<int64_t>();
    int64_t* tbaseB = tbaseA + (size_t)n_stages * (nC + 1);
    int64_t* tbaseM = tbaseB + (size_t)n_stages * (nC + 1);
    if (!p.all_narrow) {
        hipLaunchKernelGGL(k_tile_count, dim3((unsigned)nC, (unsigned)n_stages), dim3(WG_BLOCK), 0, c->sA, job.v, pa, cntA, cntB, cntM);
        HIP_TRY(hipGetLastError());
    }
    hipLaunchKernelGGL(k_stage_plan, dim3((unsigned)n_stages), dim3(WG_PLAN_BLOCK), 0, c->sA, job.v, pa, (const uint32_t*)(p.all_narrow ? nullptr : cntA),
                       (const uint32_t*)(p.all_narrow ? nullptr : cntB), (const uint32_t*)(p.all_narrow ? nullptr : cntM),
                       c->plan_cbase.as<int64_t>(), c->plan_cum0.as<uint32_t>(), tbaseA, tbaseB, tbaseM, c->plan_pairs.as<int64_t>(), c->plan_tiles.as<int64_t>());
    HIP_TRY(hipGetLastError());
    if (!p.all_narrow) {
        const bool check_div_m = c->divs_enabled && p.term_mode[2] == 2 && p.WMED > 0 && c->divs_m_pc != pc;
        int rc;
        if (check_div_m && (rc = queue_div_check(c, pc, WG_MEDIUM_WMAX, hst + 3, err, errlen)) != WGBSSEG_OK) return rc;
        HIP_TRY(hipMemcpyAsync(p.stage_pairs.data(), c->plan_pairs.p, (size_t)n_stages * 8, hipMemcpyDeviceToHost, c->sA));
        HIP_TRY(hipMemcpyAsync(p.stage_tiles.data(), c->plan_tiles.p, (size_t)n_stages * 24, hipMemcpyDeviceToHost, c->sA));
        HIP_TRY(hipStreamSynchronize(c->sA));
        if (check_div_m) {
            c->divs_m_ok = *reinterpret_cast<const unsigned int*>(&hst[3]) == 0u;
            c->divs_m_pc = pc;
            if (profiling()) fprintf(stderr, "[wgbsseg] short division core for pseudo count %g on the operand pairs of a MEDIUM tile: %s\n", (double)pc, c->divs_m_ok ? "verified on every pair" : "NOT exact, the full core stays");
        }
    }
    for (int k = 0; k < 3; k++) {
        tile0[k].assign((size_t)n_stages + 1, 0);
        for (int stg = 0; stg < n_stages; stg++) tile0[k][(size_t)stg + 1] = tile0[k][(size_t)stg] + p.stage_tiles[3 * (size_t)stg + k];
        if (tile0[k][(size_t)n_stages] > 0x7fffffffLL) { set_err(err, errlen, "too many scoring tiles in one call"); return WGBSSEG_E_ARG; }
    }
    for (int k = 0; k < 3; k++) HIP_TRY(c->tiles[k].ensure((size_t)std::max<int64_t>(1, tile0[k][(size_t)n_stages]) * sizeof(TileDesc)));
    for (int stg = 0; stg < n_stages; stg++) {
        hipLaunchKernelGGL(k_tile_emit, dim3((unsigned)nC), dim3(WG_BLOCK), 0, c->sA, job.v, pa, stg, tbaseA, tbaseB, tbaseM,
                           c->tiles[0].as<TileDesc>() + tile0[0][(size_t)stg], c->tiles[1].as<TileDesc>() + tile0[1][(size_t)stg],
                           c->tiles[2].as<TileDesc>() + tile0[2][(size_t)stg]);
        HIP_TRY(hipGetLastError());
    }
    if (p.gated) {
        HIP_TRY(c->stage_ctr.ensure((size_t)n_stages * 4));
        HIP_TRY(hipMemsetAsync(c->stage_ctr.p, 0, (size_t)n_stages * 4, c->sA));
    }
    HIP_TRY(hipEventRecord(c->ev[EV_PLAN], c->sA));
    if (p.gated) HIP_TRY(hipStreamWaitEvent(c->sA2, c->ev[EV_PLAN], 0));
    mark(4);
    return WGBSSEG_OK;
}

int Batch::stages(char* err, size_t errlen)
{
    const BatchPlan& p = plan;
    const JobView& v = job.v;
    const int n_stages = p.n_stages;
    const int64_t max_stage_pairs = std::max<int64_t>(1, *std::max_element(p.stage_pairs.begin(), p.stage_pairs.end()));
    for (int k = 0; k < p.nbuf; k++) HIP_TRY(c->cost[k].ensure((size_t)max_stage_pairs * 8));
    HIP_TRY(c->dpstate.ensure((size_t)nC * (size_t)p.state_stride * 8));
    HIP_TRY(c->tmp_borders.ensure((size_t)(job.sites_padded + nC) * 4));
    HIP_TRY(c->nb.ensure((size_t)nC * 4));
    out_head = (size_t)round_up((int64_t)(nC + 1) * 8, 16);
    c->out_par ^= 1;
    outb = &c->out_borders[c->out_par];
    HIP_TRY(outb->ensure(out_head + (size_t)(J + nC) * 4));
    for (auto* evs : {&c->ev_cost0, &c->ev_cost1, &c->ev_dp0, &c->ev_dp1, &c->ev_fork, &c->ev_join}) grow_events(*evs, n_stages);
    StageView sv;
    sv.cbase = c->plan_cbase.as<int64_t>(); sv.cum0 = c->plan_cum0.as<uint32_t>();
    sv.tbaseA = c->plan_tbase.as<int64_t>(); sv.tbaseB = sv.tbaseA + (size_t)n_stages * (nC + 1);
    sv.sb = c->plan_sb.as<int32_t>();
    DpArgs da = {p.ringN, {c->dp_wlean ? 0 : 1, 0, 0}};
#ifdef WGBSSEG_DP_TIMING
    da.pad[1] = (int)env_int("WGBSSEG_DP_DEBUG", 0);
#endif
    c->last_dp_chunks = nC; c->last_dp_stride = p.state_stride;
    const size_t lds_dp = 2 * 4096 * 8 + 128 * 8 + 64 * 12 + 16 + 1024 * 6;
    double* const dps = c->dpstate.as<double>();
    if (st.wide_units) HIP_TRY(hipStreamWaitEvent(c->sA, c->ev[EV_SCAN_END], 0));
    if (st.wide_units && p.gated) HIP_TRY(hipStreamWaitEvent(c->sA2, c->ev[EV_SCAN_END], 0));
    const bool divsA = c->divs_enabled && c->divs_ok && c->divs_pc == P.pseudo_count;
    const bool divsM = c->divs_enabled && c->divs_m_ok && c->divs_m_pc == P.pseudo_count;
    const int fast[3] = {p.term_mode[0] == 2 && divsA ? 3 : p.term_mode[0], p.term_mode[1], p.term_mode[2] == 2 && divsM ? 3 : p.term_mode[2]};
    for (int stg = 0; stg < n_stages; stg++) {
        const int64_t* const nt = &p.stage_tiles[3 * (size_t)stg];
        hipStream_t const sP = p.gated && (stg & 1) ? c->sA2 : c->sA;
        sv.stage = stg;
        double* cbuf = c->cost[stg % p.nbuf].as<double>();
        const bool side = nt[0] > 0 && (nt[1] > 0 || nt[2] > 0);
        hipStream_t const sSide = side ? (p.gated && (stg & 1) ? c->sA : c->sA2) : sP;
        if (stg >= p.nbuf) HIP_TRY(hipStreamWaitEvent(sP, c->ev_dp1[stg - p.nbuf], 0));
        if (p.gated) {
            const int64_t before = stg > 0 ? nt[-3] + nt[-2] + nt[-1] : 0;
            if (before > 0) {
                const double est_s = 10.0 * (double)p.stage_pairs[(size_t)stg - 1] * c->n_samples / 5e11;
                const long long max_ticks = (long long)(1e8 * std::min(2.0, std::max(0.005, est_s)));
                hipLaunchKernelGGL(k_stage_gate, dim3(1), dim3(64), 0, sP, (const uint32_t*)(c->stage_ctr.as<uint32_t>() + (stg - 1)),
                                   (uint32_t)std::max<int64_t>(1, before - c->stage_gate), max_ticks);
                HIP_TRY(hipGetLastError());
            }
            for (CostArgs& a : ca) a.finished = c->stage_ctr.as<uint32_t>() + stg;
        }
        HIP_TRY(hipEventRecord(c->ev_cost0[stg], sP));
        if (side) { HIP_TRY(hipEventRecord(c->ev_fork[stg], sP)); HIP_TRY(hipStreamWaitEvent(sSide, c->ev_fork[stg], 0)); }
        for (int k : {0, 2, 1})
            if (nt[k] > 0)
                HIP_TRY(launch_cost_class(k, fast[k], p.TI, v, sv, ca[k], c->tiles[k].as<TileDesc>() + tile0[k][(size_t)stg], nt[k], cbuf, p.lds[k], k == 0 ? sP : sSide));
        if (side) { HIP_TRY(hipEventRecord(c->ev_join[stg], sSide)); HIP_TRY(hipStreamWaitEvent(sP, c->ev_join[stg], 0)); }
        HIP_TRY(hipEventRecord(c->ev_cost1[stg], sP));
        HIP_TRY(hipStreamWaitEvent(c->sB, c->ev_cost1[stg], 0));
        HIP_TRY(hipEventRecord(c->ev_dp0[stg], c->sB));
        const bool dp16 = p.dp_mode == 0 && n_stages > 1 && stg + 1 < n_stages;
        if (dp16)                                  hipLaunchKernelGGL((k_dp16<3>), dim3((unsigned)nC), dim3(64 * 4), (size_t)(2 * 16 * 64 * 8 + WG_DP_META_RING * 6), c->sB, v, sv, cbuf, dps, p.state_stride);
        else if (p.dp_mode == 0 && p.all_narrow)   hipLaunchKernelGGL((k_dp<7, 64, true>), dim3((unsigned)nC), dim3(64 * 8), lds_dp, c->sB, v, sv, cbuf, da, dps, p.state_stride);
        else if (p.dp_mode == 0)                   hipLaunchKernelGGL((k_dp<7, 64>), dim3((unsigned)nC), dim3(64 * 8), lds_dp, c->sB, v, sv, cbuf, da, dps, p.state_stride);
        else if (p.dp_mode == 1)                   hipLaunchKernelGGL((k_dp<7, 32>), dim3((unsigned)nC), dim3(64 * 8), lds_dp, c->sB, v, sv, cbuf, da, dps, p.state_stride);
        else                                       hipLaunchKernelGGL((k_dp<15, 32>), dim3((unsigned)nC), dim3(64 * 16), lds_dp, c->sB, v, sv, cbuf, da, dps, p.state_stride);
        HIP_TRY(hipGetLastError());
        HIP_TRY(hipEventRecord(c->ev_dp1[stg], c->sB));
    }
    return WGBSSEG_OK;
}

int Batch::deliver(char* err, size_t errlen)
{
    int64_t* const d_boff = outb->as<int64_t>();
    int32_t* const d_bord = reinterpret_cast<int32_t*>(reinterpret_cast<char*>(outb->p) + out_head);
    HIP_TRY(hipEventRecord(c->ev[EV_TRACE0], c->sB));
    hipLaunchKernelGGL(k_trace, dim3((unsigned)nC), dim3(WG_BLOCK), 0, c->sB, job.v, c->tmp_borders.as<int32_t>(), c->nb.as<int32_t>());
    HIP_TRY(hipGetLastError());
    hipLaunchKernelGGL(k_border_offsets, dim3(1), dim3(WG_BLOCK), 0, c->sB, c->nb.as<int32_t>(), nC, d_boff);
    HIP_TRY(hipGetLastError());
    hipLaunchKernelGGL(k_gather_borders, dim3((unsigned)nC), dim3(WG_BLOCK), 0, c->sB, job.v, c->tmp_borders.as<int32_t>(), c->nb.as<int32_t>(),
                       (const int64_t*)d_boff, d_bord);
    HIP_TRY(hipGetLastError());
    HIP_TRY(hipEventRecord(c->ev[EV_TRACE1], c->sB));
    const size_t small_bytes = out_head + (size_t)(J + nC) * 4;
    const bool small = small_bytes <= (512u << 10);
    const int64_t n_lead = (early && !small && early->n_lead > 0 && early->n_lead <= nC) ? early->n_lead : 0;
    size_t rest_cap = 0;
    if (n_lead) for (int64_t i = n_lead; i < nC; i++) rest_cap += (size_t)job.h[(size_t)i].len + 1;
    const size_t edge_bytes = (size_t)n_lead * 2 * WG_EDGE * 4, rest_bytes = rest_cap * 4;
    if (n_lead) {
        HIP_TRY(c->edges.ensure(edge_bytes + rest_bytes + 16));
        hipLaunchKernelGGL(k_gather_edges, dim3((unsigned)nC), dim3(WG_BLOCK), 0, c->sB, (const int64_t*)d_boff, (const int32_t*)d_bord, (int)n_lead, c->edges.as<int32_t>(),
                           c->edges.as<int32_t>() + edge_bytes / 4);
        HIP_TRY(hipGetLastError());
        HIP_TRY(hipEventRecord(c->ev[EV_TRACE1], c->sB));
    }
    if (!c->h_out.ensure((small ? small_bytes : out_head) + edge_bytes + rest_bytes)) { set_err(err, errlen, "out of page-locked host memory"); return WGBSSEG_E_NOMEM; }
    HIP_TRY(hipMemcpyAsync(c->h_out.p, outb->p, small ? small_bytes : (size_t)(nC + 1) * 8, hipMemcpyDeviceToHost, c->sB));
    if (n_lead) HIP_TRY(hipMemcpyAsync(reinterpret_cast<char*>(c->h_out.p) + out_head, c->edges.p, edge_bytes + rest_bytes, hipMemcpyDeviceToHost, c->sB));
    if (small || n_lead) HIP_TRY(hipEventRecord(c->ev[EV_HOME], c->sB));
    mark(5);
    if (J >= (1 << 20)) {
        HIP_TRY(hipEventSynchronize(c->ev_dp1[plan.n_stages - 1]));
        wgstitch::Pool::get().heat();
    }
    HIP_TRY(hipStreamSynchronize(c->sB));
    memcpy(borders_off, c->h_out.p, (size_t)(nC + 1) * 8);
    const int64_t total_b = borders_off[nC];
    int32_t* borders_out = (*alloc)(total_b);
    if (!borders_out) { set_err(err, errlen, "borders_out too small: need %lld ints", (long long)total_b); return WGBSSEG_E_CAPACITY; }
    if (small) memcpy(borders_out, reinterpret_cast<const char*>(c->h_out.p) + out_head, (size_t)total_b * 4);
    else if (n_lead && early->dest_device_visible && (reinterpret_cast<uintptr_t>(borders_out) & 15) == 0) {
        const int64_t lead_b = borders_off[n_lead];
        HIP_TRY(hipStreamWaitEvent(c->sC, c->ev[EV_TRACE1], 0));
        hipLaunchKernelGGL(k_copy_out, dim3(512), dim3(WG_BLOCK), 0, c->sC, (const int32_t*)d_bord, borders_out, lead_b);
        HIP_TRY(hipGetLastError());
        HIP_TRY(hipEventRecord(c->evD, c->sC));
        c->out_pending = true;
        memcpy(borders_out + lead_b, reinterpret_cast<const char*>(c->h_out.p) + out_head + edge_bytes, (size_t)(total_b - lead_b) * 4);
        early->edges = reinterpret_cast<const int32_t*>(reinterpret_cast<const char*>(c->h_out.p) + out_head);
        early->pending = true;
    } else {
        HIP_TRY(hipMemcpyAsync(borders_out, d_bord, (size_t)total_b * 4, hipMemcpyDeviceToHost, c->sB));
        HIP_TRY(hipEventRecord(c->ev[EV_HOME], c->sB));
        HIP_TRY(hipStreamSynchronize(c->sB));
    }
    mark(6);
    HIP_TRY(hipEventSynchronize(c->evS));
    if (hst[2].first_bad != ~0ULL) return report_bad_site(c, hst[2], err, errlen);
    return WGBSSEG_OK;
}

int Batch::timings(char* err, size_t errlen)
{
    const int n_stages = plan.n_stages;
    const int64_t total_pairs = (int64_t)st.total_pairs;
    if (marks) {
        auto at = [&](hipEvent_t e) { float x = 0; (void)hipEventElapsedTime(&x, c->ev[EV_BEGIN], e); return (double)x; };
        if (n_stages > 1) {
            fprintf(stderr, "[wgbsseg] %d stages%s, bounds", n_stages, plan.gated ? " (gated: alternating scoring streams)" : "");
            for (int q = 0; q <= n_stages; q++) fprintf(stderr, " %d", (int)plan.sb[q]);
            fprintf(stderr, "\n");
        }
        fprintf(stderr, "[wgbsseg] batch of %d chunks, %lld sites: windows done %.3f | stats copied %.3f | scan pass (its own stream) %.3f .. %.3f | plan + tiles done %.3f | "
                "scoring %.3f .. %.3f | recurrence %.3f .. %.3f | trace %.3f .. %.3f | borders on the host %.3f\n", nC, (long long)J,
                at(c->ev[EV_WINDOWS]), at(c->ev[EV_STATS]), at(c->ev[EV_VALIDATE0]), at(c->ev[EV_SCAN_END]), at(c->ev[EV_PLAN]), at(c->ev_cost0[0]), at(c->ev_cost1[n_stages - 1]),
                at(c->ev_dp0[0]), at(c->ev_dp1[n_stages - 1]), at(c->ev[EV_TRACE0]), at(c->ev[EV_TRACE1]), at(c->ev[EV_HOME]));
    }
    wgbsseg_timings& T = c->tim;
    if (!c->accumulate) memset(&T, 0, sizeof(T));
    float ms = 0;
    if (st.wide_units) HIP_TRY(hipEventElapsedTime(&ms, c->ev[EV_SCAN0], c->ev[EV_SCAN1])); else HIP_TRY(hipEventElapsedTime(&ms, c->ev[EV_VALIDATE0], c->ev[EV_VALIDATE1]));
    T.scan_ms += ms;
    const int64_t scan_bytes = 2 * (st.wide_units ? J : job.val_sites) * c->n_samples;
    if (scan_bytes > T.scan_main_bytes) { T.scan_main_bytes = scan_bytes; T.scan_main_ms = ms; }
    HIP_TRY(hipEventElapsedTime(&ms, c->ev[EV_BEGIN], c->ev[EV_WINDOWS])); T.window_ms += ms;
    float cost_end = 0;
    for (int stg = 0; stg < n_stages; stg++) {
        float t0 = 0, t1 = 0;
        HIP_TRY(hipEventElapsedTime(&t0, c->ev[EV_BEGIN], c->ev_cost0[stg])); HIP_TRY(hipEventElapsedTime(&t1, c->ev[EV_BEGIN], c->ev_cost1[stg]));
        if (t1 > std::max(t0, cost_end)) T.cost_ms += t1 - std::max(t0, cost_end);
        cost_end = std::max(cost_end, t1);
        HIP_TRY(hipEventElapsedTime(&ms, c->ev_dp0[stg], c->ev_dp1[stg])); T.dp_ms += ms;
    }
    HIP_TRY(hipEventElapsedTime(&ms, c->ev[EV_TRACE0], c->ev[EV_TRACE1])); T.trace_ms += ms;
    HIP_TRY(hipEventElapsedTime(&ms, c->ev[EV_BEGIN], c->ev[EV_HOME])); T.total_ms += ms;
    T.sites += J; T.pairs += total_pairs; T.evals += total_pairs * c->n_samples;
    T.scan_bytes += scan_bytes; T.max_window = std::max<int32_t>(T.max_window, plan.Wmax);
    T.n_stages = std::max<int32_t>(T.n_stages, n_stages); T.scan_launches += 1;
    if (plan.term_mode[0] == 2 && c->divs_enabled && c->divs_ok && c->divs_pc == P.pseudo_count) T.div_short = 1;
    c->last_sites = J; c->last_pairs = total_pairs; c->last_stages = n_stages; c->last_valid = true;
    c->batch_open = false;
    if (marks) {
        hm[7] = wall_s();
        fprintf(stderr, "[wgbsseg]   host clock of the batch, us after entry: tables up %.0f | windows queued %.0f | statistics here %.0f | scoring's tiles queued %.0f | everything queued %.0f | results here %.0f | return %.0f\n",
                (hm[1] - hm[0]) * 1e6, (hm[2] - hm[0]) * 1e6, (hm[3] - hm[0]) * 1e6, (hm[4] - hm[0]) * 1e6, (hm[5] - hm[0]) * 1e6, (hm[6] - hm[0]) * 1e6, (hm[7] - hm[0]) * 1e6);
    }
    return WGBSSEG_OK;
}

}

extern "C" {

int wgbsseg_segment_chunks(wgbsseg_ctx* c, const int64_t* chunk_start0, const int32_t* chunk_len, int64_t n_chunks,
                           const wgbsseg_params* P, int32_t* borders_out, int64_t borders_cap, int64_t* borders_off,
                           char* err, size_t errlen)
{
    if (!borders_out) { set_err(err, errlen, "NULL borders pointer"); return WGBSSEG_E_ARG; }
    BorderAlloc alloc = [&](int64_t total) -> int32_t* { return total <= borders_cap ? borders_out : nullptr; };
    return segment_chunks_impl(c, chunk_start0, chunk_len, n_chunks, P, alloc, borders_off, err, errlen);
}

int wgbsseg_segment_chunks_host(const uint8_t* betas, int64_t n_samples, int64_t sample_pitch_bytes, int64_t n_sites_total,
                                const uint32_t* loci, const int64_t* chunk_start0, const int32_t* chunk_len, int64_t n_chunks,
                                const wgbsseg_params* params, int device, int32_t* borders_out, int64_t borders_cap,
                                int64_t* borders_off, char* err, size_t errlen)
{
    if (!betas || n_samples < 1 || sample_pitch_bytes < 2 * n_sites_total) { set_err(err, errlen, "bad beta buffer"); return WGBSSEG_E_ARG; }
    wgbsseg_ctx* c = nullptr;
    int rc = wgbsseg_create(device, &c, err, errlen);
    if (rc != WGBSSEG_OK) return rc;
    std::vector<const uint8_t*> ptrs((size_t)n_samples);
    for (int64_t s = 0; s < n_samples; s++) ptrs[(size_t)s] = betas + s * sample_pitch_bytes;
    rc = wgbsseg_set_betas_host(c, ptrs.data(), n_samples, n_sites_total, err, errlen);
    if (rc == WGBSSEG_OK) rc = wgbsseg_set_loci_host(c, loci, n_sites_total, err, errlen);
    if (rc == WGBSSEG_OK) rc = wgbsseg_segment_chunks(c, chunk_start0, chunk_len, n_chunks, params, borders_out, borders_cap, borders_off, err, errlen);
    wgbsseg_destroy(c);
    return rc;
}

}

namespace {
int run_ctx_batch(wgbsseg_ctx* c, const std::vector<int64_t>& st0, const std::vector<int32_t>& ln, const wgbsseg_params* P, int64_t slot,
                  bool accumulate, const int32_t*& flat, std::vector<int64_t>& off, std::unique_ptr<int32_t[]>& owned, std::string& msg, EarlyOut* early = nullptr)
{
    off.resize(st0.size() + 1);
    int32_t* dst = nullptr;
    BorderAlloc alloc = [&](int64_t total) -> int32_t* {
        if (c->pinned.size() <= (size_t)slot) c->pinned.resize((size_t)slot + 1);
        PinnedBuf& pb = c->pinned[(size_t)slot];
        dst = pb.ensure((size_t)std::max<int64_t>(total, 1) * 4) ? reinterpret_cast<int32_t*>(pb.p) : nullptr;
        if (early) early->dest_device_visible = dst != nullptr;
        if (!dst) { owned.reset(new int32_t[(size_t)std::max<int64_t>(total, 1)]); dst = owned.get(); }
        return dst;
    };
    char ebuf[512] = {0};
    const bool acc_before = c->accumulate;
    c->accumulate = accumulate;
// ... 660 lines not shown
    if (rc) { set_err(err, errlen, "%s", msg.c_str()); return WGBSSEG_E_ARG; }
    return WGBSSEG_OK;
}

int wgbsseg_blocks_write_bedgraph(const char* path, const char* text, const int64_t* line_off, const int32_t* len3, int64_t n_rows,
                                  const void* rows, int32_t wide, int32_t threads, char* err, size_t errlen)
{
    if (!path || n_rows < 0 || (n_rows && (!text || !line_off || !len3 || !rows))) { set_err(err, errlen, "write_bedgraph: bad argument"); return WGBSSEG_E_ARG; }
    int64_t base = 0;
    const int fd = open_for_rows(path, 0, &base, err, errlen);
    if (fd < 0) return WGBSSEG_E_ARG;
    const wgtab::Rows R = {text, line_off, len3, nullptr, nullptr, nullptr};
    std::string msg;
    const int rc = wide ? wgtab::write_bedgraph<uint16_t>(fd, base, R, n_rows, static_cast<const uint16_t*>(rows), threads, msg)
                        : wgtab::write_bedgraph<uint8_t>(fd, base, R, n_rows, static_cast<const uint8_t*>(rows), threads, msg);
    if (close(fd) != 0 && rc == 0) { set_err(err, errlen, "write to %s failed", path); return WGBSSEG_E_ARG; }
    if (rc) { set_err(err, errlen, "%s", msg.c_str()); return WGBSSEG_E_ARG; }
    return WGBSSEG_OK;
}

int wgbsseg_bed_parse(const char* text, int64_t len, int64_t cap, const char* const* chrom_names, int32_t n_chroms, int64_t* line_off,
                      int32_t* len3, int32_t* row_len, int32_t* chrom, int64_t* start, int64_t* end, int64_t* n_rows, int32_t* width, int32_t* header)
{
    if (!n_rows || !width || !header) return WGBSSEG_E_ARG;
    *n_rows = 0; *width = 0; *header = 0;
    if (!text || len < 0 || cap < 0 || n_chroms < 0 || (n_chroms && !chrom_names) || (cap && (!line_off || !len3 || !row_len || !chrom || !start || !end))) return WGBSSEG_E_ARG;
    const int rc = wgtab::parse_bed(text, len, cap, chrom_names, n_chroms, line_off, len3, row_len, chrom, start, end, n_rows, width, header);
    return rc == 0 ? WGBSSEG_OK : (rc == 1 ? 1 : WGBSSEG_E_ARG);
}

int64_t wgbsseg_debug_canonical_float(const char* tokens, int64_t len, uint8_t* out, int64_t out_cap)
{
    if (!tokens || len < 0 || !out) return -1;
    int64_t n = 0;
    for (int64_t a = 0; a < len;) {
        const char* nl = static_cast<const char*>(memchr(tokens + a, '\n', (size_t)(len - a)));
        const int64_t b = nl ? (int64_t)(nl - tokens) : len;
        if (n >= out_cap) return -1;
        out[n++] = wgtab::canonical_float(tokens + a, (size_t)(b - a)) ? 1 : 0;
        a = b + 1;
    }
    return n;
}

int wgbsseg_bed_write_annotated(const char* path, const char* text, const int64_t* line_off, const int32_t* len3, const int32_t* row_len,
                                const int64_t* start_cpg, const int64_t* end_cpg, int64_t n_rows, int32_t threads, char* err, size_t errlen)
{
    if (n_rows < 0 || (n_rows && (!text || !line_off || !len3 || !row_len || !start_cpg || !end_cpg))) { set_err(err, errlen, "bed_write_annotated: bad argument"); return WGBSSEG_E_ARG; }
    int64_t base = -1;
    const int fd = path ? open_for_rows(path, 0, &base, err, errlen) : 1;
    if (fd < 0) return WGBSSEG_E_ARG;
    std::string msg;
    const int rc = wgtab::write_annotated_bed(fd, base, text, line_off, len3, row_len, start_cpg, end_cpg, n_rows, threads, msg);
    if (path && close(fd) != 0 && rc == 0) { set_err(err, errlen, "write to %s failed", path); return WGBSSEG_E_ARG; }
    if (rc) { set_err(err, errlen, "%s", msg.c_str()); return WGBSSEG_E_ARG; }
    return WGBSSEG_OK;
}

int64_t wgbsseg_format_fixed(const double* v, int64_t n, int32_t digits, char* out, int64_t out_cap)
{
    if (n < 0 || (n && (!v || !out))) return -1;
    char* p = out;
    for (int64_t i = 0; i < n; i++) {
        if (out_cap - (p - out) < 420) return -1;
        p = wgtab::put_fixed(p, v[i], digits);
        *p++ = '\n';
    }
    return (int64_t)(p - out);
}

}

#include "pat_engines.h"

extern "C" {

int wgbsseg_get_timings(const wgbsseg_ctx* c, wgbsseg_timings* out)
{
    if (!c || !out) return WGBSSEG_E_ARG;
    *out = c->tim;
    return WGBSSEG_OK;
}

int64_t wgbsseg_debug_fetch(wgbsseg_ctx* c, const char* what, void* out, int64_t cap_bytes)
{
    if (!c || !what || !out || !c->last_valid) return WGBSSEG_E_STATE;
    const void* src = nullptr;
    int64_t bytes = 0;
    if (!strcmp(what, "window")) { src = c->W16.p; bytes = c->last_sites * 2; }
    else if (!strcmp(what, "cum")) { src = c->cum32.p; bytes = c->last_sites * 4; }
    else if (!strcmp(what, "back")) { src = c->back16.p; bytes = c->last_sites * 2; }
    else if (!strcmp(what, "dpstate")) { src = c->dpstate.p; bytes = c->last_dp_chunks * c->last_dp_stride * 8; }
    else if (!strcmp(what, "cost")) { if (c->last_stages != 1) return WGBSSEG_E_STATE; src = c->cost[0].p; bytes = c->last_pairs * 8; }
    else return WGBSSEG_E_ARG;
    if (bytes > cap_bytes) return WGBSSEG_E_CAPACITY;
    if (hipSetDevice(c->device) != hipSuccess) return WGBSSEG_E_HIP;
    if (hipMemcpy(out, src, (size_t)bytes, hipMemcpyDeviceToHost) != hipSuccess) return WGBSSEG_E_HIP;
    return bytes;
}

int wgbsseg_debug_sample_terms(wgbsseg_ctx* c, const float* nmeth, const float* ntotal, int64_t count, float pseudo_count, float* out)
{
    char* err = nullptr; size_t errlen = 0;
    if (!c || !nmeth || !ntotal || !out || count < 1) return WGBSSEG_E_ARG;
    HIP_TRY(hipSetDevice(c->device));
    HIP_TRY(c->dbg_a.ensure((size_t)count * 4)); HIP_TRY(c->dbg_b.ensure((size_t)count * 4)); HIP_TRY(c->dbg_c.ensure((size_t)count * 4));
    HIP_TRY(hipMemcpyAsync(c->dbg_a.p, nmeth, (size_t)count * 4, hipMemcpyHostToDevice, c->sA));
    HIP_TRY(hipMemcpyAsync(c->dbg_b.p, ntotal, (size_t)count * 4, hipMemcpyHostToDevice, c->sA));
    const unsigned blocks = (unsigned)std::min<int64_t>((count + 255) / 256, 8192);
    const int fast = wg_term_mode(pseudo_count);
    const int rows = fast == 2 ? wg_lookup_rows(pseudo_count, 255.0 * 8000) : 0;
    if (rows > WG_KY_KMIN + 1) return WGBSSEG_E_ARG;
    hipLaunchKernelGGL(k_debug_terms, dim3(blocks), dim3(256), 0, c->sA, c->dbg_a.as<float>(), c->dbg_b.as<float>(), count, pseudo_count, c->dbg_c.as<float>(), fast, rows);
    HIP_TRY(hipGetLastError());
    HIP_TRY(hipMemcpyAsync(out, c->dbg_c.p, (size_t)count * 4, hipMemcpyDeviceToHost, c->sA));
    HIP_TRY(hipStreamSynchronize(c->sA));
    return WGBSSEG_OK;
}

int wgbsseg_debug_div(wgbsseg_ctx* c, const float* a, const float* b, int64_t count, uint32_t* out_fast, uint32_t* out_ieee)
{
    char* err = nullptr; size_t errlen = 0;
    if (!c || !a || !b || !out_fast || !out_ieee || count < 1) return WGBSSEG_E_ARG;
    HIP_TRY(hipSetDevice(c->device));
    HIP_TRY(c->dbg_a.ensure((size_t)count * 8)); HIP_TRY(c->dbg_b.ensure((size_t)count * 8));
    float* da = c->dbg_a.as<float>(); float* db = da + count;
    uint32_t* o1 = c->dbg_b.as<uint32_t>(); uint32_t* o2 = o1 + count;
    HIP_TRY(hipMemcpyAsync(da, a, (size_t)count * 4, hipMemcpyHostToDevice, c->sA));
    HIP_TRY(hipMemcpyAsync(db, b, (size_t)count * 4, hipMemcpyHostToDevice, c->sA));
    const unsigned blocks = (unsigned)std::min<int64_t>((count + 255) / 256, 16384);
    hipLaunchKernelGGL(k_debug_div, dim3(blocks), dim3(256), 0, c->sA, da, db, count, o1, o2);
    HIP_TRY(hipGetLastError());
    HIP_TRY(hipMemcpyAsync(out_fast, o1, (size_t)count * 4, hipMemcpyDeviceToHost, c->sA));
    HIP_TRY(hipMemcpyAsync(out_ieee, o2, (size_t)count * 4, hipMemcpyDeviceToHost, c->sA));
    HIP_TRY(hipStreamSynchronize(c->sA));
    return WGBSSEG_OK;
}

int wgbsseg_debug_div_short(wgbsseg_ctx* c, const float* a, const float* b, int64_t count, uint32_t* out)
{
    char* err = nullptr; size_t errlen = 0;
    if (!c || !a || !b || !out || count < 1) return WGBSSEG_E_ARG;
    HIP_TRY(hipSetDevice(c->device));
    HIP_TRY(c->dbg_a.ensure((size_t)count * 8)); HIP_TRY(c->dbg_b.ensure((size_t)count * 4));
    float* da = c->dbg_a.as<float>(); float* db = da + count;
    HIP_TRY(hipMemcpyAsync(da, a, (size_t)count * 4, hipMemcpyHostToDevice, c->sA));
    HIP_TRY(hipMemcpyAsync(db, b, (size_t)count * 4, hipMemcpyHostToDevice, c->sA));
    const unsigned blocks = (unsigned)std::min<int64_t>((count + 255) / 256, 16384);
    hipLaunchKernelGGL(k_debug_div_short, dim3(blocks), dim3(256), 0, c->sA, da, db, count, c->dbg_b.as<uint32_t>());
    HIP_TRY(hipGetLastError());
    HIP_TRY(hipMemcpyAsync(out, c->dbg_b.p, (size_t)count * 4, hipMemcpyDeviceToHost, c->sA));
    HIP_TRY(hipStreamSynchronize(c->sA));
    return WGBSSEG_OK;
}

int wgbsseg_debug_check_div(wgbsseg_ctx* c, float pseudo_count, int32_t max_total, int64_t* mismatches)
{
    char* err = nullptr; size_t errlen = 0;
    if (!c || !mismatches || max_total < 0 || max_total > (1 << 21)) return WGBSSEG_E_ARG;
    HIP_TRY(hipSetDevice(c->device));
    HIP_TRY(c->divcheck.ensure(4));
    HIP_TRY(hipMemsetAsync(c->divcheck.p, 0, 4, c->sA));
    hipLaunchKernelGGL(k_check_div, dim3((unsigned)max_total + 1), dim3(WG_BLOCK), 0, c->sA, pseudo_count, pseudo_count + pseudo_count,
                       (int)max_total, c->divcheck.as<unsigned int>());
    HIP_TRY(hipGetLastError());
    unsigned int n = 0;
// ... 27 lines not shown
```

Measured before the change: 1.123 billion.

## Speculatively launch narrow-tile scoring before host reads window statistics

```diff
diff --git a/include/wgbsseg.h b/include/wgbsseg.h
--- a/include/wgbsseg.h
+++ b/include/wgbsseg.h
@@ -8,7 +8,7 @@
 extern "C" {
 #endif
 
-#define WGBSSEG_VERSION 290
+#define WGBSSEG_VERSION 291
 #define WGBSSEG_MAX_CPG 65535
 
 #define WGBSSEG_OK              0
@@ -243,6 +243,8 @@
 
 int wgbsseg_get_timings(const wgbsseg_ctx* ctx, wgbsseg_timings* out);
 
+int wgbsseg_front_speculation(const wgbsseg_ctx* ctx, int64_t* counts);
+
 int64_t wgbsseg_debug_fetch(wgbsseg_ctx* ctx, const char* what, void* out, int64_t cap_bytes);
 int wgbsseg_debug_sample_terms(wgbsseg_ctx* ctx, const float* nmeth, const float* ntotal, int64_t count,
                                float pseudo_count, float* out);
diff --git a/wgbs_tools_amd/_lib.py b/wgbs_tools_amd/_lib.py
--- a/wgbs_tools_amd/_lib.py
+++ b/wgbs_tools_amd/_lib.py
@@ -14,7 +14,7 @@
 
 OK, E_ARG, E_METH_GT_COV, E_NOMEM, E_HIP, E_LOCI_ORDER, E_CAPACITY, E_STATE, E_IO = 0, -1, -2, -3, -4, -5, -6, -7, -8
 
-ABI_VERSION = 290
+ABI_VERSION = 291
 EXPORTS = ['wgbsseg_version', 'wgbsseg_device_count', 'wgbsseg_create', 'wgbsseg_destroy',
            'wgbsseg_set_betas_host', 'wgbsseg_set_betas_device', 'wgbsseg_set_loci_host', 'wgbsseg_set_loci_device',
            'wgbsseg_segment_chunks', 'wgbsseg_segment_regions', 'wgbsseg_segment_chunks_host', 'wgbsseg_prefix_sums', 'wgbsseg_scan_only',
@@ -36,7 +36,8 @@
            'wgbsseg_beta2bed', 'wgbsseg_beta2bed_pass_ms', 'wgbsseg_beta2bed_limits',
            'wgbsseg_site_counts', 'wgbsseg_site_table', 'wgbsseg_site_table_pass_ms', 'wgbsseg_site_table_limits',
            'wgbsseg_patbeta_feed_bgzf', 'wgbsseg_homog_feed_bgzf', 'wgbsseg_bimodal_feed_bgzf',
-           'wgbsseg_patbeta_inflate_ms', 'wgbsseg_homog_inflate_ms', 'wgbsseg_bimodal_inflate_ms', 'wgbsseg_bgzf_inflate']
+           'wgbsseg_patbeta_inflate_ms', 'wgbsseg_homog_inflate_ms', 'wgbsseg_bimodal_inflate_ms', 'wgbsseg_bgzf_inflate',
+           'wgbsseg_front_speculation']
 
 
 class NativeLibraryError(RuntimeError):
@@ -156,6 +157,8 @@
     L.wgbsseg_scan_only.argtypes = [vp, vp, vp, i64, i32, i32, C.POINTER(C.c_double), C.POINTER(i64), C.POINTER(i64), C.c_char_p, C.c_size_t]
     L.wgbsseg_get_timings.restype = i32
     L.wgbsseg_get_timings.argtypes = [vp, C.POINTER(Timings)]
+    L.wgbsseg_front_speculation.restype = i32
+    L.wgbsseg_front_speculation.argtypes = [vp, C.POINTER(C.c_int64)]
     L.wgbsseg_debug_fetch.restype = i64
     L.wgbsseg_debug_fetch.argtypes = [vp, C.c_char_p, vp, i64]
     L.wgbsseg_debug_sample_terms.restype = i32
@@ -562,6 +565,11 @@
         self._L.wgbsseg_get_timings(self._h, C.byref(t))
         return t.as_dict()
 
+    def front_speculation(self):
+        n = (C.c_int64 * 3)()
+        self._L.wgbsseg_front_speculation(self._h, n)
+        return int(n[0]), int(n[1]), int(n[2])
+
     def debug_fetch(self, what, dtype, count):
         out = np.empty(count, dtype=dtype)
         got = self._L.wgbsseg_debug_fetch(self._h, what.encode(), out.ctypes.data, out.nbytes)
diff --git a/wgbs_tools_amd/csrc/seg_kernels.h b/wgbs_tools_amd/csrc/seg_kernels.h
--- a/wgbs_tools_amd/csrc/seg_kernels.h
+++ b/wgbs_tools_amd/csrc/seg_kernels.h
@@ -528,7 +528,7 @@
             const int64_t s0 = P.sb[stg];
             if (s0 < cd.len) {
                 const int64_t s1 = (P.sb[stg + 1] < cd.len) ? P.sb[stg + 1] : cd.len;
-                c0 = J.cum32[cd.site_off + s0];
+                c0 = s0 > 0 ? J.cum32[cd.site_off + s0] : 0u;
                 const uint64_t cend = (s1 < cd.len) ? (uint64_t)J.cum32[cd.site_off + s1] : (uint64_t)J.chunk_pairs[c];
                 sz = cend - c0;
                 nt = cntA ? (uint64_t)cntA[(int64_t)stg * nC + c] : (uint64_t)((s1 - s0 + P.TI - 1) / P.TI);
@@ -613,6 +613,19 @@
     }
 }
 
+__global__ __launch_bounds__(WG_BLOCK) void k_tile_emit_narrow(JobView J, int ti, const int64_t* __restrict__ tbase, TileDesc* __restrict__ tiles)
+{
+    const int c = blockIdx.x;
+    const ChunkDesc cd = J.chunks[c];
+    const int64_t t0 = tbase[c];
+    const int nU = (cd.len + ti - 1) / ti;
+    for (int u = threadIdx.x; u < nU; u += WG_BLOCK) {
+        const int ka = u * ti;
+        const TileDesc d = {c, ka, cd.len - ka < ti ? cd.len - ka : ti, 0};
+        tiles[t0 + u] = d;
+    }
+}
+
 struct CostArgs {
     float pc, pc2;
     int32_t NS;
@@ -621,7 +634,15 @@
     int32_t xcd_group;
     int32_t cmap;
     uint32_t* finished;
+    const JobStatus* guard;
+    unsigned long long guard_pairs;
 };
+
+__host__ __device__ __forceinline__ bool wg_speculation_holds(unsigned int max_window, unsigned long long total_pairs, unsigned int loci_disorder, unsigned int overflow,
+                                                              unsigned long long cap_pairs)
+{
+    return max_window <= (unsigned int)WG_NARROW_WMAX && total_pairs <= cap_pairs && loci_disorder == 0u && overflow == 0u;
+}
 
 __global__ __launch_bounds__(64) void k_stage_gate(const uint32_t* __restrict__ finished, uint32_t need, long long max_ticks)
 {
@@ -827,6 +848,7 @@
     const int64_t G = A.xcd_group, jx = (int64_t)(blockIdx.x >> 3);
     const int64_t t = (jx / G) * (8 * G) + (int64_t)(blockIdx.x & 7) * G + (jx % G);
     if (t >= n_tiles) return;
+    if (A.guard != nullptr && !wg_speculation_holds(A.guard->max_window, A.guard->total_pairs, A.guard->loci_disorder, A.guard->overflow, A.guard_pairs)) return;
     const TileDesc td = tiles[t];
     const int c = td.chunk;
     const ChunkDesc cd = J.chunks[c];
diff --git a/wgbs_tools_amd/csrc/wgbsseg.hip b/wgbs_tools_amd/csrc/wgbsseg.hip
--- a/wgbs_tools_amd/csrc/wgbsseg.hip
+++ b/wgbs_tools_amd/csrc/wgbsseg.hip
@@ -151,6 +151,9 @@
     int64_t scan_piece_sites = 4096;
     int medium_wmax = WG_MEDIUM_WMAX;
     bool dp_wlean = true, early = true, speculate = true, batch_marks = false;
+    bool front_spec = true;
+    double favg_hint[2] = {0.0, 0.0};
+    int64_t n_batches = 0, n_speculated = 0, n_spec_held = 0;
     ~wgbsseg_ctx() { (void)hipSetDevice(device); (void)hipDeviceSynchronize(); }
 };
 
@@ -420,6 +423,7 @@
     c->dp_wlean = env_flag("WGBSSEG_DP_WLEAN", true);
     c->early = !env_flag("WGBSSEG_NO_EARLY", false);
     c->speculate = !env_flag("WGBSSEG_NO_SPECULATION", false);
+    c->front_spec = !env_flag("WGBSSEG_NO_FRONT_SPECULATION", false);
     c->batch_marks = env_int("WGBSSEG_PROFILE", 0) >= 2;
     g_live_ctx[device & 63].fetch_add(1, std::memory_order_relaxed);
     c->counted_live = true;
@@ -521,11 +525,12 @@
     int64_t sites_padded = 0;
     int32_t max_len = 0;
     JobStatus st0;
+    int64_t spec_tbase_at = 0, spec_sb_at = 0, spec_tiles = 0;
     JobView v = {};
 };
 
 int build_job(wgbsseg_ctx* c, const int64_t* start0, const int32_t* len, int64_t n_chunks, Job& job, bool need_loci,
-              char* err, size_t errlen)
+              char* err, size_t errlen, int spec_ti = 0)
 {
     if (!c) { set_err(err, errlen, "ctx is NULL"); return WGBSSEG_E_ARG; }
     if (!c->betas) { set_err(err, errlen, "betas not set"); return WGBSSEG_E_STATE; }
@@ -563,6 +568,17 @@
             while (cix + 1 < n_chunks && job.wtile_off[(size_t)cix + 1] <= tile) cix++;
             hint[h] = (int32_t)cix;
         }
+    }
+    if (spec_ti > 0) {
+        job.spec_tbase_at = (int64_t)job.wtile_off.size();
+        job.spec_sb_at = job.spec_tbase_at + n_chunks + 1;
+        job.wtile_off.resize((size_t)job.spec_sb_at + 1);
+        int64_t* tb = job.wtile_off.data() + job.spec_tbase_at;
+        tb[0] = 0;
+        for (int64_t i = 0; i < n_chunks; i++) tb[i + 1] = tb[i] + (len[i] + spec_ti - 1) / spec_ti;
+        job.spec_tiles = tb[n_chunks];
+        const int32_t sb[2] = {0, job.max_len};
+        memcpy(job.wtile_off.data() + job.spec_sb_at, sb, sizeof sb);
     }
     job.sites = total; job.sites_padded = so; job.carry_entries = co; job.units = uo;
     HIP_TRY(hipSetDevice(c->device));
@@ -957,7 +973,19 @@
     bool marks = false;
     double hm[8] = {0, 0, 0, 0, 0, 0, 0, 0};
     void mark(int i) { if (marks) hm[i] = wall_s(); }
-
+    struct Speculation {
+        bool on = false, held = false;
+        const char* why = "off";
+        int TI = 0, NS = 0, fast = 0, rows = 0;
+        size_t lds = 0;
+        unsigned long long cap_pairs = 0;
+        bool beside = false;
+    } spec;
+    const int32_t* d_sb = nullptr;
+
+    void plan_speculation();
+    int speculate(char* err, size_t errlen);
+    void reconcile();
     int front(char* err, size_t errlen);
     int disorder_exit(char* err, size_t errlen);
     int tile_plan(char* err, size_t errlen);
@@ -993,7 +1021,8 @@
         c->out_pending = false;
     }
     if (c) c->batch_open = true;
-    int rc = build_job(c, chunk_start0, chunk_len, n_chunks, b.job, true, err, errlen);
+    b.plan_speculation();
+    int rc = build_job(c, chunk_start0, chunk_len, n_chunks, b.job, true, err, errlen, b.spec.on ? b.spec.TI : 0);
     if (rc != WGBSSEG_OK) return rc;
     rc = plan_validation(c, b.job, !c->accumulate, err, errlen);
     if (rc != WGBSSEG_OK) return rc;
@@ -1007,11 +1036,104 @@
     rc = plan_tiles(c, b.job, b.st, b.P.pseudo_count, b.plan, err, errlen);
     if (rc != WGBSSEG_OK) return rc;
     plan_stages(c, b.job, b.st, b.plan);
+    c->favg_hint[b.J >= (1 << 20)] = (double)(int64_t)b.st.total_pairs / (double)std::max<int64_t>(1, b.J);
+    b.reconcile();
     rc = b.tile_plan(err, errlen);
     if (rc == WGBSSEG_OK) rc = b.stages(err, errlen);
     if (rc == WGBSSEG_OK) rc = b.deliver(err, errlen);
     if (rc == WGBSSEG_OK) rc = b.timings(err, errlen);
     return rc;
+}
+
+void Batch::plan_speculation()
+{
+    spec = Speculation();
+    if (!c) return;
+    c->n_batches++;
+    if (!c->front_spec) { spec.why = "switched off"; return; }
+    if (c->force_stages > 1 || c->force_dp_mode != 0) { spec.why = "stages or recurrence forced"; return; }
+    const size_t cap_bytes = std::min<size_t>(c->cost[0].cap, (size_t)c->cost_budget_bytes);
+    if (!c->cost[0].p || cap_bytes < 8) { spec.why = "no cost buffer yet"; return; }
+    if (!chunk_len || n_chunks < 1 || n_chunks > 0x7fffffff) { spec.why = "bad chunk list"; return; }
+    int64_t sites = 0;
+    int32_t max_len = 0;
+    int n_long = 0;
+    for (int64_t i = 0; i < n_chunks; i++) {
+        if (chunk_len[i] < 1 || chunk_len[i] > (1 << 30)) { spec.why = "bad chunk list"; return; }
+        sites += chunk_len[i]; max_len = std::max(max_len, chunk_len[i]); n_long += chunk_len[i] >= 8192;
+    }
+    if (max_len >= 8192 && n_long <= 160) { spec.why = "few long chunks: the statistics decide on stages"; return; }
+    const float pc = P.pseudo_count;
+    const int tm = wg_term_mode(pc);
+    if (tm == 2 && c->divs_enabled && c->divs_pc != pc) { spec.why = "the division core is not verified for this pseudo count yet"; return; }
+    JobStatus guess = {};
+    guess.max_window = std::min<uint32_t>(P.max_cpg, WG_NARROW_WMAX);
+    const int cls = sites >= (1 << 20);
+    const double hint = c->favg_hint[cls] > 0 ? c->favg_hint[cls] : (c->favg_hint[1 - cls] > 0 ? c->favg_hint[1 - cls] : 20.0);
+    guess.total_pairs = (unsigned long long)(std::min<double>(hint, guess.max_window) * (double)sites);
+    Job shape;
+    shape.sites = sites;
+    BatchPlan form;
+    char e[8];
+    if (plan_tiles(c, shape, guess, pc, form, e, sizeof e) != WGBSSEG_OK) { spec.why = "no tile form"; return; }
+    if (tm == 2 && !(c->lookup.p && c->lookup_pc == pc && c->lookup_rows[0] == form.rows[0])) { spec.why = "lookup tables not on the device yet"; return; }
+    spec.on = true; spec.why = "";
+    spec.TI = form.TI; spec.NS = form.NS[0]; spec.rows = form.rows[0]; spec.lds = form.lds[0];
+    spec.fast = tm == 2 && c->divs_enabled && c->divs_ok ? 3 : tm;
+    spec.cap_pairs = cap_bytes / 8;
+    spec.beside = sites >= (1 << 20);
+}
+
+int Batch::speculate(char* err, size_t errlen)
+{
+    const int64_t* const d_wtile = c->wtile.as<int64_t>();
+    d_sb = reinterpret_cast<const int32_t*>(d_wtile + job.spec_sb_at);
+    hipStream_t const sP = spec.beside ? c->sA2 : c->sA;
+    if (spec.beside) HIP_TRY(hipStreamWaitEvent(sP, c->ev[EV_UPLOADED], 0));
+    hipLaunchKernelGGL(k_tile_emit_narrow, dim3((unsigned)nC), dim3(WG_BLOCK), 0, sP, job.v, spec.TI, d_wtile + job.spec_tbase_at, c->tiles[0].as<TileDesc>());
+    HIP_TRY(hipGetLastError());
+    PlanArgs pa = {d_sb, spec.TI, WG_NARROW_WMAX, WG_WIDE_TK, 1, c->medium_wmax};
+    int64_t* tbaseA = c->plan_tbase.as<int64_t>();
+    int64_t* tbaseB = tbaseA + (nC + 1);
+    int64_t* tbaseM = tbaseB + (nC + 1);
+    if (spec.beside) HIP_TRY(hipStreamWaitEvent(sP, c->ev[EV_WINDOWS], 0));
+    hipLaunchKernelGGL(k_stage_plan, dim3(1), dim3(WG_PLAN_BLOCK), 0, sP, job.v, pa, (const uint32_t*)nullptr, (const uint32_t*)nullptr, (const uint32_t*)nullptr,
+                       c->plan_cbase.as<int64_t>(), c->plan_cum0.as<uint32_t>(), tbaseA, tbaseB, tbaseM, c->plan_pairs.as<int64_t>(), c->plan_tiles.as<int64_t>());
+    HIP_TRY(hipGetLastError());
+    HIP_TRY(hipEventRecord(c->ev[EV_PLAN], sP));
+    if (spec.beside) HIP_TRY(hipStreamWaitEvent(c->sA, c->ev[EV_PLAN], 0));
+    for (auto* evs : {&c->ev_cost0, &c->ev_cost1, &c->ev_dp0, &c->ev_dp1, &c->ev_fork, &c->ev_join}) grow_events(*evs, 1);
+    StageView sv;
+    sv.cbase = c->plan_cbase.as<int64_t>(); sv.cum0 = c->plan_cum0.as<uint32_t>();
+    sv.tbaseA = tbaseA; sv.tbaseB = tbaseB;
+    sv.stage = 0; sv.sb = d_sb;
+    CostArgs a;
+    memset(&a, 0, sizeof(a));
+    a.pc = P.pseudo_count; a.pc2 = P.pseudo_count + P.pseudo_count;
+    a.NS = spec.NS; a.rows = spec.rows;
+    a.tab = spec.fast >= 2 ? c->lookup.as<wg_d2>() : nullptr;
+    a.xcd_group = 64; a.cmap = 3;
+    a.guard = c->status.as<JobStatus>(); a.guard_pairs = spec.cap_pairs;
+    HIP_TRY(hipEventRecord(c->ev_cost0[0], c->sA));
+    HIP_TRY(launch_cost_class(0, spec.fast, spec.TI, job.v, sv, a, c->tiles[0].as<TileDesc>(), job.spec_tiles, c->cost[0].as<double>(), spec.lds, c->sA));
+    HIP_TRY(hipEventRecord(c->ev_cost1[0], c->sA));
+    c->n_speculated++;
+    return WGBSSEG_OK;
+}
+
+void Batch::reconcile()
+{
+    if (!spec.on) return;
+    if (!wg_speculation_holds(st.max_window, st.total_pairs, st.loci_disorder, st.overflow, spec.cap_pairs))
+        spec.why = st.max_window > (unsigned int)WG_NARROW_WMAX ? "a window beyond the narrow tiles'" : "more scored blocks than the cost buffer held";
+    else if (!plan.all_narrow || plan.n_stages != 1 || plan.gated) spec.why = "the plan is staged";
+    else {
+        spec.held = true;
+        spec.why = plan.TI == spec.TI && plan.NS[0] == spec.NS ? "" : "with the guessed tile form, not the one the statistics choose";
+        plan.TI = spec.TI; plan.NS[0] = spec.NS; plan.lds[0] = spec.lds;
+        plan.stage_tiles[0] = job.spec_tiles;
+        c->n_spec_held++;
+    }
 }
 
 int Batch::front(char* err, size_t errlen)
@@ -1049,6 +1171,15 @@
     const int64_t win_want = 1 + (int64_t)WG_WIN_TILE + 2 * (int64_t)std::max(top_step, 32) + 8;
     const int win_lds = win_want <= 12288 ? (int)win_want : 0;
     const int64_t* const d_wtile = c->wtile.as<int64_t>();
+    if (spec.on && job.spec_tiles + 8 * 64 > 0x7fffffffLL) { spec.on = false; spec.why = "too many scoring tiles"; }
+    if (spec.on) {
+        HIP_TRY(c->tiles[0].ensure((size_t)std::max<int64_t>(1, job.spec_tiles) * sizeof(TileDesc)));
+        HIP_TRY(c->plan_cbase.ensure((size_t)nC * 8));
+        HIP_TRY(c->plan_cum0.ensure((size_t)nC * 4));
+        HIP_TRY(c->plan_tbase.ensure((size_t)(nC + 1) * 8 * 3));
+        HIP_TRY(c->plan_pairs.ensure(8));
+        HIP_TRY(c->plan_tiles.ensure(8 * 3));
+    }
     hipLaunchKernelGGL(k_window, dim3((unsigned)nT), dim3(WG_BLOCK), (size_t)win_lds * 4, c->sA, v, c->status.as<JobStatus>(),
                        d_wtile, reinterpret_cast<const int32_t*>(d_wtile + nC + 1), P.max_cpg, P.max_bp, win_lds, top_step, std::max(c->medium_wmax, WG_NARROW_WMAX),
                        c->tile_tot.as<uint32_t>(), c->tile_chunk.as<int4>());
@@ -1056,11 +1187,14 @@
     hipLaunchKernelGGL(k_window_scan, dim3((unsigned)nC), dim3(WG_BLOCK), 0, c->sA, v, c->status.as<JobStatus>(), d_wtile, c->tile_tot.as<uint32_t>(), c->tile_base.as<uint32_t>());
     HIP_TRY(hipGetLastError());
     HIP_TRY(hipEventRecord(c->ev[EV_WINDOWS], c->sA));
-    HIP_TRY(hipMemcpyAsync(&hst[0], c->status.p, sizeof(JobStatus), hipMemcpyDeviceToHost, c->sA));
-    HIP_TRY(hipEventRecord(c->ev[EV_STATS], c->sA));
+    hipStream_t const sStats = spec.on && spec.beside ? c->sB : c->sA;
+    if (sStats != c->sA) HIP_TRY(hipStreamWaitEvent(sStats, c->ev[EV_WINDOWS], 0));
+    HIP_TRY(hipMemcpyAsync(&hst[0], c->status.p, sizeof(JobStatus), hipMemcpyDeviceToHost, sStats));
+    HIP_TRY(hipEventRecord(c->ev[EV_STATS], sStats));
     hipLaunchKernelGGL(k_window_cum, dim3((unsigned)((nT + WG_CUM_TILES - 1) / WG_CUM_TILES)), dim3(WG_BLOCK), 0, c->sA, (const uint16_t*)v.W16, v.cum32, (const int4*)c->tile_chunk.as<int4>(),
                        (const uint32_t*)c->tile_base.as<uint32_t>(), nT);
     HIP_TRY(hipGetLastError());
+    if (spec.on && (rc = speculate(err, errlen)) != WGBSSEG_OK) return rc;
     mark(2);
     HIP_TRY(hipEventSynchronize(c->ev[EV_STATS]));
     mark(3);
@@ -1143,6 +1277,7 @@
 int Batch::tile_plan(char* err, size_t errlen)
 {
     BatchPlan& p = plan;
+    if (spec.held) { mark(4); return WGBSSEG_OK; }
     const float pc = P.pseudo_count;
     const int n_stages = p.n_stages;
     CostArgs base;
@@ -1175,6 +1310,7 @@
     const void* src = p.sb;
     if (c->h_sb.ensure(sb_bytes)) { memcpy(c->h_sb.p, src, sb_bytes); src = c->h_sb.p; }
     HIP_TRY(hipMemcpyAsync(c->plan_sb.p, src, sb_bytes, hipMemcpyHostToDevice, c->sA));
+    d_sb = c->plan_sb.as<int32_t>();
     HIP_TRY(c->plan_cbase.ensure((size_t)n_stages * nC * 8));
     HIP_TRY(c->plan_cum0.ensure((size_t)n_stages * nC * 4));
     HIP_TRY(c->plan_tbase.ensure((size_t)n_stages * (nC + 1) * 8 * 3));
@@ -1249,7 +1385,7 @@
     StageView sv;
     sv.cbase = c->plan_cbase.as<int64_t>(); sv.cum0 = c->plan_cum0.as<uint32_t>();
     sv.tbaseA = c->plan_tbase.as<int64_t>(); sv.tbaseB = sv.tbaseA + (size_t)n_stages * (nC + 1);
-    sv.sb = c->plan_sb.as<int32_t>();
+    sv.sb = d_sb;
     DpArgs da = {p.ringN, {c->dp_wlean ? 0 : 1, 0, 0}};
 #ifdef WGBSSEG_DP_TIMING
     da.pad[1] = (int)env_int("WGBSSEG_DP_DEBUG", 0);
@@ -1281,13 +1417,15 @@
             }
             for (CostArgs& a : ca) a.finished = c->stage_ctr.as<uint32_t>() + stg;
         }
-        HIP_TRY(hipEventRecord(c->ev_cost0[stg], sP));
-        if (side) { HIP_TRY(hipEventRecord(c->ev_fork[stg], sP)); HIP_TRY(hipStreamWaitEvent(sSide, c->ev_fork[stg], 0)); }
-        for (int k : {0, 2, 1})
-            if (nt[k] > 0)
-                HIP_TRY(launch_cost_class(k, fast[k], p.TI, v, sv, ca[k], c->tiles[k].as<TileDesc>() + tile0[k][(size_t)stg], nt[k], cbuf, p.lds[k], k == 0 ? sP : sSide));
-        if (side) { HIP_TRY(hipEventRecord(c->ev_join[stg], sSide)); HIP_TRY(hipStreamWaitEvent(sP, c->ev_join[stg], 0)); }
-        HIP_TRY(hipEventRecord(c->ev_cost1[stg], sP));
+        if (!spec.held) {
+            HIP_TRY(hipEventRecord(c->ev_cost0[stg], sP));
+            if (side) { HIP_TRY(hipEventRecord(c->ev_fork[stg], sP)); HIP_TRY(hipStreamWaitEvent(sSide, c->ev_fork[stg], 0)); }
+            for (int k : {0, 2, 1})
+                if (nt[k] > 0)
+                    HIP_TRY(launch_cost_class(k, fast[k], p.TI, v, sv, ca[k], c->tiles[k].as<TileDesc>() + tile0[k][(size_t)stg], nt[k], cbuf, p.lds[k], k == 0 ? sP : sSide));
+            if (side) { HIP_TRY(hipEventRecord(c->ev_join[stg], sSide)); HIP_TRY(hipStreamWaitEvent(sP, c->ev_join[stg], 0)); }
+            HIP_TRY(hipEventRecord(c->ev_cost1[stg], sP));
+        }
         HIP_TRY(hipStreamWaitEvent(c->sB, c->ev_cost1[stg], 0));
         HIP_TRY(hipEventRecord(c->ev_dp0[stg], c->sB));
         const bool dp16 = p.dp_mode == 0 && n_stages > 1 && stg + 1 < n_stages;
@@ -1370,15 +1508,19 @@
     const int64_t total_pairs = (int64_t)st.total_pairs;
     if (marks) {
         auto at = [&](hipEvent_t e) { float x = 0; (void)hipEventElapsedTime(&x, c->ev[EV_BEGIN], e); return (double)x; };
+        char front[256];
+        if (spec.on) snprintf(front, sizeof front, "%s%s%s (TI %d, NS %d, room for %llu scored blocks, %llu needed)", spec.held ? "held" : "NOT held: ",
+                              spec.held && spec.why[0] ? " " : "", spec.why, spec.TI, spec.NS, spec.cap_pairs, (unsigned long long)st.total_pairs);
+        else snprintf(front, sizeof front, "none (%s)", spec.why);
         if (n_stages > 1) {
             fprintf(stderr, "[wgbsseg] %d stages%s, bounds", n_stages, plan.gated ? " (gated: alternating scoring streams)" : "");
             for (int q = 0; q <= n_stages; q++) fprintf(stderr, " %d", (int)plan.sb[q]);
             fprintf(stderr, "\n");
         }
         fprintf(stderr, "[wgbsseg] batch of %d chunks, %lld sites: windows done %.3f | stats copied %.3f | scan pass (its own stream) %.3f .. %.3f | plan + tiles done %.3f | "
-                "scoring %.3f .. %.3f | recurrence %.3f .. %.3f | trace %.3f .. %.3f | borders on the host %.3f\n", nC, (long long)J,
+                "scoring %.3f .. %.3f | recurrence %.3f .. %.3f | trace %.3f .. %.3f | borders on the host %.3f | front speculation: %s\n", nC, (long long)J,
                 at(c->ev[EV_WINDOWS]), at(c->ev[EV_STATS]), at(c->ev[EV_VALIDATE0]), at(c->ev[EV_SCAN_END]), at(c->ev[EV_PLAN]), at(c->ev_cost0[0]), at(c->ev_cost1[n_stages - 1]),
-                at(c->ev_dp0[0]), at(c->ev_dp1[n_stages - 1]), at(c->ev[EV_TRACE0]), at(c->ev[EV_TRACE1]), at(c->ev[EV_HOME]));
+                at(c->ev_dp0[0]), at(c->ev_dp1[n_stages - 1]), at(c->ev[EV_TRACE0]), at(c->ev[EV_TRACE1]), at(c->ev[EV_HOME]), front);
     }
     wgbsseg_timings& T = c->tim;
     if (!c->accumulate) memset(&T, 0, sizeof(T));
@@ -2205,6 +2347,13 @@
     return WGBSSEG_OK;
 }
 
+int wgbsseg_front_speculation(const wgbsseg_ctx* c, int64_t* counts)
+{
+    if (!c || !counts) return WGBSSEG_E_ARG;
+    counts[0] = c->n_batches; counts[1] = c->n_speculated; counts[2] = c->n_spec_held;
+    return WGBSSEG_OK;
+}
+
 int64_t wgbsseg_debug_fetch(wgbsseg_ctx* c, const char* what, void* out, int64_t cap_bytes)
 {
     if (!c || !what || !out || !c->last_valid) return WGBSSEG_E_STATE;
```

Measured after the change: 1.122 billion, median of 2. No clear change (-0.1%).
